# nexus-xyz/nexus-zkvm

Measured on AMD Instinct MI355X. Metric: RISC-V cycles proved/sec at log_n_rows=22; achieved HBM GB/s on Circle-FFT, higher is better.
Workload: dtype u32 (M31); 1 GPU; synthetic 2^22-row trace, full prove (LDE+quotient+FRI+Merkle), 27 preprocessed + 347 main + 64 interaction columns (16 real logup columns generated on device, recorded AIR), blowup 2, 3 queries, pow_bits 10, standard Blake2s-256 Merkle nodes; log_n_rows=22, parallelism=1 GPU, proof_words=11971

## Files before the change

### nexus-zkvm_amd/csrc/ctx.hip

```cpp
#include "internal.h"
#include <execinfo.h>
#include <signal.h>
#include <unistd.h>
#include <string.h>
#include <stdlib.h>
#include <algorithm>
#include <thread>

namespace nx {

thread_local std::string g_last_error;

int set_err(nx_ctx* ctx, int code, const std::string& msg) {
    g_last_error = msg;
    if (ctx) ctx->err = msg;
    return code;
}
int hip_fail(nx_ctx* ctx, hipError_t e, const char* what, const char* file, int line) {
    char buf[512];
    snprintf(buf, sizeof buf, "HIP error %d (%s) in `%s` at %s:%d", (int)e, hipGetErrorString(e), what, file, line);
    return set_err(ctx, e == hipErrorOutOfMemory ? NX_ERR_OOM : NX_ERR_HIP, buf);
}

int stage(nx_ctx* ctx, const void* h_src, size_t bytes, void** d_out) {
// ... 214 lines not shown

__global__ __launch_bounds__(256) void transpose_blocks_kernel(uint32_t* full, uint64_t col_stride, uint32_t* blocks, uint32_t n_cols, uint64_t rows, uint32_t world, int unpack) {
    const uint64_t rb4 = rows / world / 4, total = (uint64_t)n_cols * world * rb4;
    for (uint64_t i = blockIdx.x * (uint64_t)blockDim.x + threadIdx.x; i < total; i += (uint64_t)gridDim.x * blockDim.x) {
        const uint64_t x = i % rb4, cd = i / rb4;
        const uint32_t c = (uint32_t)(cd % n_cols), d = (uint32_t)(cd / n_cols);
        uint4* f = reinterpret_cast<uint4*>(full + (uint64_t)c * col_stride) + (uint64_t)d * rb4 + x;
        uint4* b = reinterpret_cast<uint4*>(blocks) + ((uint64_t)d * n_cols + c) * rb4 + x;
        if (unpack) *f = *b; else *b = *f;
    }
}
int transpose_blocks(nx_ctx* ctx, uint32_t* full, uint64_t col_stride, uint32_t* blocks, uint32_t n_cols, uint64_t rows, uint32_t world, bool unpack) {
    if (!n_cols || !rows) return NX_OK;
    if ((rows / world) % 4 || rows % world || col_stride % 4) return set_err(ctx, NX_ERR_ARG, "transpose_blocks: the row block must be a multiple of 4 words");
    const uint64_t total = (uint64_t)n_cols * rows / 4;
    hipLaunchKernelGGL(transpose_blocks_kernel, dim3((unsigned)std::min<uint64_t>((total + 255) / 256, (uint64_t)ctx->n_cus * 32)), dim3(256), 0, ctx->stream, full, col_stride, blocks, n_cols,
                       rows, world, unpack ? 1 : 0);
    NX_LAUNCH_CHECK(ctx);
    return NX_OK;
}

}

using namespace nx;

__global__ __launch_bounds__(256) void copy_cols_kernel(nx::ColSet dst, nx::ColSet src, size_t n4) {
    const uint4* __restrict__ s = (const uint4*)src.col(blockIdx.y);
    uint4* __restrict__ d = (uint4*)dst.col(blockIdx.y);
    for (size_t i = (size_t)blockIdx.x * 256 + threadIdx.x; i < n4; i += (size_t)gridDim.x * 256) d[i] = s[i];
}
namespace nx {
int copy_columns(nx_ctx* ctx, uint32_t* const* h_dst, const uint32_t* const* h_src, uint32_t n_cols, size_t n_words) {
    if (n_cols == 0 || n_words == 0) return NX_OK;
    bool vec = (n_words & 3) == 0;
    for (uint32_t k = 0; k < n_cols && vec; k++) vec = !(((uintptr_t)h_dst[k] | (uintptr_t)h_src[k]) & 15);
    if (!vec || n_cols < 4) { for (uint32_t k = 0; k < n_cols; k++) NX_TRY(nx_copy(ctx, h_dst[k], h_src[k], n_words)); return NX_OK; }
    for (uint32_t c0 = 0; c0 < n_cols; c0 += 65535) {
        const uint32_t nb = std::min<uint32_t>(65535, n_cols - c0);
        ColSet d, s;
        NX_TRY(make_colset(ctx, h_dst + c0, nb, &d));
        NX_TRY(make_colset(ctx, (uint32_t* const*)(h_src + c0), nb, &s));
        const size_t n4 = n_words / 4;
        const unsigned bx = (unsigned)std::max<size_t>(1, std::min<size_t>((n4 + 255) / 256, std::max<size_t>(1, (size_t)ctx->n_cus * 16 / nb)));
        hipLaunchKernelGGL(copy_cols_kernel, dim3(bx, nb), dim3(256), 0, ctx->stream, d, s, n4);
        NX_LAUNCH_CHECK(ctx);
    }
    return NX_OK;
}
}

extern "C" {

const char* nx_version(void) { return "nexus_hip 0.3 (gfx950)"; }

const char* nx_last_error(const nx_ctx* ctx) { return ctx ? ctx->err.c_str() : g_last_error.c_str(); }

static int env_int(const char* name, int dflt) { const char* e = getenv(name); return e ? atoi(e) : dflt; }
static int clampi(int v, int lo, int hi) { return v < lo ? lo : v > hi ? hi : v; }
static nx_options options_from_env() {
    nx_options o;
    o.fft_batch_cols = std::max(1, env_int("NX_FFT_BATCH", 2));
    o.fft_streams = clampi(env_int("NX_FFT_STREAMS", 2), 1, 4);
    o.fri_dist_min_log = std::max(0, env_int("NX_FRI_DIST_MIN_LOG", 21));
    o.dist_chunks = std::max(0, env_int("NX_DIST_CHUNKS", 0));
    o.air_segment = std::max(200, env_int("NX_AIR_SEGMENT", 9000));
    o.air_degree_split = env_int("NX_AIR_DEGREE_SPLIT", 1) != 0;
    o.quotients_coeffs = env_int("NX_QUOTIENTS_COEFFS", 1) != 0;
    o.air_half_domain = env_int("NX_AIR_HALF_DOMAIN", 1) != 0;
    o.air_quarter_domain = std::max(0, std::min(2, env_int("NX_AIR_QUARTER_DOMAIN", 2)));
    o.comm_timeout_ms = std::max(0, env_int("NX_COMM_TIMEOUT_MS", 120000));
    o.fft_kmax = clampi(env_int("NX_FFT_KMAX", 9), 1, 11);
    o.fft_fused = env_int("NX_FFT_FUSED", 1) != 0;
    o.merkle_fused = clampi(env_int("NX_MERKLE_FUSED", 21), 0, 31);
    o.merkle_subtree = clampi(env_int("NX_MERKLE_SUBTREE", 14), 0, 30);
    o.merkle_top = clampi(env_int("NX_MERKLE_TOP", 7), 1, 10);
    o.merkle_pair_levels = env_int("NX_MERKLE_PAIR_LEVELS", 1) != 0;
    o.fri_device_channel = env_int("NX_FRI_DEVICE_CHANNEL", 1) != 0;
    o.fri_tail = clampi(env_int("NX_FRI_TAIL", 1), 0, 11);
    o.logup_scan_tiled = env_int("NX_LOGUP_SCAN_TILED", 1) != 0;
    o.logup_per_column = env_int("NX_LOGUP_PER_COLUMN", 0) != 0;
    o.machine_reuse_pre = env_int("NX_MACHINE_REUSE_PREPROCESSED", 0) != 0;
    o.machine_logup_program = env_int("NX_MACHINE_LOGUP_PROGRAM", 0) != 0;
    o.trace_vec4 = env_int("NX_TRACE_VEC4", 1) != 0;
    o.host_pack_threads = clampi((int)std::thread::hardware_concurrency(), 1, 16);
    return o;
}
struct OptEntry { const char* name; int nx_options::*field; int lo, hi; };
static const OptEntry k_options[] = {
    {"fft.batch_cols", &nx_options::fft_batch_cols, 1, 256},
    {"fft.streams", &nx_options::fft_streams, 1, 4},
    {"fri.dist_min_log", &nx_options::fri_dist_min_log, 0, 31},
    {"dist.chunks", &nx_options::dist_chunks, 0, 64},
    {"air.segment", &nx_options::air_segment, 200, 1 << 30},
    {"air.degree_split", &nx_options::air_degree_split, 0, 1},
    {"quotients.coeffs", &nx_options::quotients_coeffs, 0, 1},
    {"air.half_domain", &nx_options::air_half_domain, 0, 1},
    {"air.quarter_domain", &nx_options::air_quarter_domain, 0, 2},
    {"comm.timeout_ms", &nx_options::comm_timeout_ms, 0, 1 << 30},
    {"fft.kmax", &nx_options::fft_kmax, 1, 11},
    {"fft.fused", &nx_options::fft_fused, 0, 1},
    {"merkle.fused", &nx_options::merkle_fused, 0, 31},
    {"merkle.subtree", &nx_options::merkle_subtree, 0, 30},
    {"merkle.top", &nx_options::merkle_top, 1, 10},
    {"merkle.pair_levels", &nx_options::merkle_pair_levels, 0, 1},
    {"fri.device_channel", &nx_options::fri_device_channel, 0, 1},
    {"fri.tail", &nx_options::fri_tail, 0, 11},
    {"logup.scan_tiled", &nx_options::logup_scan_tiled, 0, 1},
    {"logup.per_column", &nx_options::logup_per_column, 0, 1},
    {"machine.reuse_preprocessed", &nx_options::machine_reuse_pre, 0, 1},
    {"machine.logup_program", &nx_options::machine_logup_program, 0, 1},
    {"trace.vec4", &nx_options::trace_vec4, 0, 1},
    {"host.pack_threads", &nx_options::host_pack_threads, 1, 64},
};
int nx_ctx_set_option(nx_ctx* ctx, const char* name, int64_t value) {
    if (!ctx || !name) return set_err(ctx, NX_ERR_ARG, "nx_ctx_set_option: NULL argument");
    for (const OptEntry& e : k_options)
        if (!strcmp(e.name, name)) {
            if (value < e.lo || value > e.hi) return set_err(ctx, NX_ERR_ARG, std::string("nx_ctx_set_option: value out of range for ") + name);
            ctx->opt.*(e.field) = (int)value;
            return NX_OK;
        }
    return set_err(ctx, NX_ERR_ARG, std::string("nx_ctx_set_option: unknown option ") + name);
}
int nx_ctx_get_option(const nx_ctx* ctx, const char* name, int64_t* value) {
    if (!ctx || !name || !value) return set_err(const_cast<nx_ctx*>(ctx), NX_ERR_ARG, "nx_ctx_get_option: NULL argument");
    for (const OptEntry& e : k_options)
        if (!strcmp(e.name, name)) { *value = ctx->opt.*(e.field); return NX_OK; }
    return set_err(const_cast<nx_ctx*>(ctx), NX_ERR_ARG, std::string("nx_ctx_get_option: unknown option ") + name);
}

static void abort_backtrace(int sig) {
    void* frames[64];
    const int n = backtrace(frames, 64);
    static const char msg[] = "\n[nexus_hip] SIGABRT — native stack of the aborting thread:\n";
    (void)!write(2, msg, sizeof msg - 1);
    backtrace_symbols_fd(frames, n, 2);
    signal(sig, SIG_DFL);
    raise(sig);
}
int nx_ctx_create(int device, nx_ctx** out) {
    if (!out) return set_err(nullptr, NX_ERR_ARG, "nx_ctx_create: out is NULL");
    { static bool once = false; if (!once) { once = true; const char* e = getenv("NX_ABORT_BACKTRACE"); if (e && *e == '1') signal(SIGABRT, abort_backtrace); } }
    int count = 0;
    hipError_t e = hipGetDeviceCount(&count);
    if (e != hipSuccess || count <= 0)
        return set_err(nullptr, NX_ERR_NO_DEVICE, "nx_ctx_create: no HIP device visible (this library has no CPU fallback)");
    if (device < 0 || device >= count) return set_err(nullptr, NX_ERR_ARG, "nx_ctx_create: bad device index");
    hipDeviceProp_t prop;
    NX_HIP(nullptr, hipGetDeviceProperties(&prop, device));
    if (!strstr(prop.gcnArchName, "gfx950"))
        return set_err(nullptr, NX_ERR_NO_DEVICE, std::string("nx_ctx_create: device is ") + prop.gcnArchName + ", this library is built for gfx950 only");
    NX_HIP(nullptr, hipSetDevice(device));
    nx_ctx* c = new nx_ctx();
    c->opt = options_from_env();
    c->device = device; c->hash_mode = NX_HASH_BLAKE2S; c->timing = false; c->n_cus = prop.multiProcessorCount > 0 ? prop.multiProcessorCount : 256;
    c->scratch_size = 16u << 20; c->scratch_off = 0; c->d_scratch = nullptr; c->h_scratch = nullptr; c->cached_bytes = 0;
    for (int i = 0; i < 4; i++) { c->kind_ms[i] = 0; c->kind_bytes[i] = 0; }
    NX_HIP(nullptr, hipStreamCreateWithFlags(&c->stream, hipStreamNonBlocking));
    c->cur = c->stream;
    NX_HIP(nullptr, hipStreamCreateWithFlags(&c->copy_stream, hipStreamNonBlocking));
    NX_HIP(nullptr, hipStreamCreateWithFlags(&c->perm_stream, hipStreamNonBlocking));
    NX_HIP(nullptr, hipEventCreateWithFlags(&c->fork_ev, hipEventDisableTiming));
    for (int i = 0; i < 3; i++) {
        NX_HIP(nullptr, hipStreamCreateWithFlags(&c->side[i], hipStreamNonBlocking));
        NX_HIP(nullptr, hipEventCreateWithFlags(&c->join_ev[i], hipEventDisableTiming));
    }
    NX_HIP(nullptr, hipMalloc((void**)&c->d_scratch, c->scratch_size));
    NX_HIP(nullptr, hipHostMalloc((void**)&c->h_scratch, c->scratch_size, hipHostMallocDefault));
    *out = c;
    return NX_OK;
}

void nx_ctx_destroy(nx_ctx* ctx) {
    NX_GUARD(ctx);
    if (!ctx) return;
    (void)hipSetDevice(ctx->device);
    (void)hipStreamSynchronize(ctx->stream);
    nxhip::machine_kernels_release(ctx);
    nx::logup_kernels_release(ctx);
    timing_flush(ctx);
    for (auto e : ctx->event_pool) (void)hipEventDestroy(e);
    dev_cache_release(ctx);
    for (auto& kv : ctx->live_blocks) (void)hipFree(kv.first);
    if (ctx->d_scratch) (void)hipFree(ctx->d_scratch);
    if (ctx->h_scratch) (void)hipHostFree(ctx->h_scratch);
    if (ctx->h_bounce) { (void)hipHostFree(ctx->h_bounce); for (int k = 0; k < 2; k++) (void)hipEventDestroy(ctx->bounce_ev[k]); }
    pack_ring_release(ctx);
    for (auto& kv : ctx->free_pinned) (void)hipHostFree(kv.second);
    for (auto& kv : ctx->live_pinned) (void)hipHostFree(kv.first);
    for (int i = 0; i < 3; i++) { (void)hipStreamDestroy(ctx->side[i]); (void)hipEventDestroy(ctx->join_ev[i]); }
    (void)hipEventDestroy(ctx->fork_ev);
    (void)hipStreamDestroy(ctx->copy_stream); (void)hipStreamDestroy(ctx->perm_stream);
    (void)hipStreamDestroy(ctx->stream);
    delete ctx;
}

int nx_ctx_set_hash_mode(nx_ctx* ctx, int mode) {
    if (!ctx) return set_err(nullptr, NX_ERR_ARG, "nx_ctx_set_hash_mode: NULL context");
    if (mode != NX_HASH_BLAKE2S && mode != NX_HASH_BLAKE2S_RAW0) return set_err(ctx, NX_ERR_ARG, "bad hash mode");
    ctx->hash_mode = mode;
    return NX_OK;
}

int nx_sync(nx_ctx* ctx) { NX_GUARD(ctx); if (!ctx) return set_err(nullptr, NX_ERR_ARG, "nx_sync: NULL context"); NX_HIP(ctx, hipStreamSynchronize(ctx->stream)); return NX_OK; }
int nx_ctx_trim(nx_ctx* ctx) { NX_GUARD(ctx); if (!ctx) return set_err(nullptr, NX_ERR_ARG, "nx_ctx_trim: NULL context"); NX_TRY(nx_sync(ctx)); dev_cache_release(ctx); pack_ring_release(ctx); return NX_OK; }
void* nx_ctx_stream(nx_ctx* ctx) { return ctx ? (void*)ctx->stream : nullptr; }
int nx_ctx_memory(nx_ctx* ctx, uint64_t* live_bytes, uint64_t* peak_bytes, int reset_peak) {
    if (!ctx) return set_err(nullptr, NX_ERR_ARG, "nx_ctx_memory: NULL context");
    if (live_bytes) *live_bytes = ctx->live_bytes;
    if (peak_bytes) *peak_bytes = ctx->peak_live_bytes;
    if (reset_peak) ctx->peak_live_bytes = ctx->live_bytes;
    return NX_OK;
}

int nx_alloc(nx_ctx* ctx, size_t n_words, uint32_t** d_out) {
    NX_GUARD(ctx);
    if (!ctx || !d_out) return set_err(ctx, NX_ERR_ARG, "nx_alloc: NULL argument");
    *d_out = nullptr;
    return dev_alloc(ctx, n_words * 4, (void**)d_out);
}
int nx_free(nx_ctx* ctx, uint32_t* d_ptr) {
    NX_GUARD(ctx);
    if (!ctx) return set_err(nullptr, NX_ERR_ARG, "nx_free: NULL context");
    dev_free(ctx, d_ptr);
    return NX_OK;
}
int nx_memset_zero(nx_ctx* ctx, uint32_t* d_ptr, size_t n_words) {
    NX_GUARD(ctx);
    if (!ctx || (!d_ptr && n_words)) return set_err(ctx, NX_ERR_ARG, "nx_memset_zero: NULL argument");
    if (!n_words) return NX_OK;
    NX_HIP(ctx, hipMemsetAsync(d_ptr, 0, n_words * 4, ctx->stream));
    return NX_OK;
}
int nx_upload(nx_ctx* ctx, uint32_t* d_dst, const uint32_t* h_src, size_t n_words) {
    NX_GUARD(ctx);
    if (!ctx || ((!d_dst || !h_src) && n_words)) return set_err(ctx, NX_ERR_ARG, "nx_upload: NULL argument");
    if (!n_words) return NX_OK;
    return copy_h2d_blocking(ctx, d_dst, h_src, n_words * 4);
}
int nx_download(nx_ctx* ctx, uint32_t* h_dst, const uint32_t* d_src, size_t n_words) {
    NX_GUARD(ctx);
    if (!ctx || ((!h_dst || !d_src) && n_words)) return set_err(ctx, NX_ERR_ARG, "nx_download: NULL argument");
    if (!n_words) return NX_OK;
    return copy_d2h_blocking(ctx, h_dst, d_src, n_words * 4);
}

int nx_copy(nx_ctx* ctx, uint32_t* d_dst, const uint32_t* d_src, size_t n_words) {
    NX_GUARD(ctx);
    if (!ctx || ((!d_dst || !d_src) && n_words)) return set_err(ctx, NX_ERR_ARG, "nx_copy: NULL argument");
    if (n_words == 0) return NX_OK;
    if ((n_words & 3) || ((uintptr_t)d_dst & 15) || ((uintptr_t)d_src & 15)) {
        NX_HIP(ctx, hipMemcpyAsync(d_dst, d_src, n_words * 4, hipMemcpyDeviceToDevice, ctx->stream));
        return NX_OK;
    }
    size_t n4 = n_words / 4;
    unsigned blocks = (unsigned)std::min<size_t>((n4 + 255) / 256, (size_t)ctx->n_cus * 16);
    hipLaunchKernelGGL(copy_kernel, dim3(blocks), dim3(256), 0, ctx->stream, (uint4*)d_dst, (const uint4*)d_src, n4);
    NX_LAUNCH_CHECK(ctx);
    return NX_OK;
}

static unsigned stream_grid(nx_ctx* ctx, size_t n) { return (unsigned)std::min<size_t>((n + 255) / 256, (size_t)ctx->n_cus * 16); }
int nx_m31_add_into(nx_ctx* ctx, uint32_t* d_dst, const uint32_t* d_src, size_t n_words) {
    NX_GUARD(ctx);
    if (!n_words) return NX_OK;
    hipLaunchKernelGGL(m31_add_into_kernel, dim3(stream_grid(ctx, n_words)), dim3(256), 0, ctx->stream, d_dst, d_src, n_words);
    NX_LAUNCH_CHECK(ctx);
    return NX_OK;
}
int nx_m31_widen(nx_ctx* ctx, uint64_t* d_dst, const uint32_t* d_src, size_t n_words) {
    NX_GUARD(ctx);
    if (!n_words) return NX_OK;
    hipLaunchKernelGGL(m31_widen_kernel, dim3(stream_grid(ctx, n_words)), dim3(256), 0, ctx->stream, (u64*)d_dst, d_src, n_words);
    NX_LAUNCH_CHECK(ctx);
    return NX_OK;
}
int nx_m31_narrow(nx_ctx* ctx, uint32_t* d_dst, const uint64_t* d_src, size_t n_words) {
    NX_GUARD(ctx);
    if (!n_words) return NX_OK;
    hipLaunchKernelGGL(m31_narrow_kernel, dim3(stream_grid(ctx, n_words)), dim3(256), 0, ctx->stream, d_dst, (const u64*)d_src, n_words);
    NX_LAUNCH_CHECK(ctx);
    return NX_OK;
}

int nx_gather(nx_ctx* ctx, const uint32_t* const* d_ptrs, const uint64_t* index, size_t n, uint32_t* h_out) {
    NX_GUARD(ctx);
    if (!ctx || ((!d_ptrs || !index || !h_out) && n)) return set_err(ctx, NX_ERR_ARG, "nx_gather: NULL argument");
    if (n == 0) return NX_OK;
// ... 24 lines not shown
```

### nexus-zkvm_amd/csrc/fft.hip

```cpp
#include "internal.h"
#include "host/narrow_pack.h"
#include <mutex>
#include <atomic>
#include <stdlib.h>
#include <algorithm>

namespace nx {

__global__ void twiddle_kernel(u32* tw, u32* itw, int h, GenTable gen) {
    u32 p = blockIdx.x * blockDim.x + threadIdx.x;
    u32 total = 1u << h;
    if (p >= total) return;
    u32 q = total - p;
    u32 val;
    if (q == 1) {
        val = 1;
    } else {
        int m = 31 - __clz(q - 1);
        int l = h - 1 - m;
        u32 k = (2u << m) - q;
        u32 init = (1u << (31 - h - 2)) << l, step = (1u << (31 - h)) << l;
        u32 idx = (init + step * bitrev(k, m)) & 0x7fffffffu;
        val = pt_from_index_tbl(gen, idx).x;
    }
// ... 250 lines not shown
}

static int check_tw(nx_ctx* ctx, const nx_twiddles* tw, int n) {
    if (!tw) return set_err(ctx, NX_ERR_ARG, "twiddles are NULL");
    if (n < 1 || n - 1 > (int)tw->log_half) return set_err(ctx, NX_ERR_ARG, "domain larger than the twiddle tree (or log_size < 1)");
    return NX_OK;
}

static int interpolate_cols(nx_ctx* ctx, const nx_twiddles* tw, ColSet cols, u32 n_cols, int n) {
    if (n >= 13 && !g_tune.legacy) return fft13_interpolate(ctx, tw, cols, n_cols, n);
    if (n <= 2) {
        hipLaunchKernelGGL(fft_tiny_kernel, dim3((n_cols + 63) / 64), dim3(64), 0, ctx->cur, cols, cols, n_cols, n, n, true);
        NX_LAUNCH_CHECK(ctx);
        return NX_OK;
    }
    std::vector<PassPlan> plan = plan_passes(n);
    u32 scale = m_inv(1u << n);
    for (size_t i = 0; i < plan.size(); i++) {
        FftPass a; a.src = cols; a.dst = cols; a.tw = tw->d_itw; a.tw_log = tw->log_half; a.n = n; a.log_in = n;
        a.lo = plan[i].lo; a.hi = plan[i].hi; a.B = plan[i].B; a.scale = i + 1 == plan.size() ? scale : 0; a.n_cols = n_cols;
        NX_TRY(launch_pass(ctx, true, a));
    }
    return NX_OK;
}

static int evaluate_cols(nx_ctx* ctx, const nx_twiddles* tw, ColSet polys, u32 n_cols, int log_in, int n, ColSet out) {
    if (log_in >= 13 && !g_tune.legacy) return fft13_evaluate(ctx, tw, polys, n_cols, log_in, n, out);
    if (n <= 2) {
        hipLaunchKernelGGL(fft_tiny_kernel, dim3((n_cols + 63) / 64), dim3(64), 0, ctx->cur, polys, out, n_cols, n, log_in, false);
        NX_LAUNCH_CHECK(ctx);
        return NX_OK;
    }
    std::vector<PassPlan> plan = plan_passes(n);
    for (size_t k = plan.size(); k-- > 0;) {
        bool first = k + 1 == plan.size();
        FftPass a; a.src = first ? polys : out; a.dst = out; a.tw = tw->d_tw; a.tw_log = tw->log_half; a.n = n;
        a.log_in = first ? log_in : n; a.lo = plan[k].lo; a.hi = plan[k].hi; a.B = plan[k].B; a.scale = 0; a.n_cols = n_cols;
        NX_TRY(launch_pass(ctx, false, a));
    }
    return NX_OK;
}

static u32 batch_for(const nx_ctx* ctx, uint32_t log_size) {
    if (log_size > 22) return (u32)std::max(1, ctx->opt.fft_batch_cols >> std::min<uint32_t>(log_size - 22, 8));
    const int shift = log_size < 22 ? (int)(22 - log_size) : 0;
    return (u32)std::min<uint64_t>((uint64_t)ctx->opt.fft_batch_cols << std::min(shift, 8), 256);
}

int fft_interpolate(nx_ctx* ctx, const nx_twiddles* tw, ColSet cols, uint32_t n_cols, uint32_t log_size) {
    NX_TRY(check_tw(ctx, tw, (int)log_size));
    tune_init();
    KTimer t(ctx, NX_T_LDE, (uint64_t)n_cols * 8ull << log_size);
    const u32 bc = batch_for(ctx, log_size);
    const int ns = n_cols > bc ? ctx->opt.fft_streams : 1;
    NX_TRY(streams_fork(ctx, ns));
    int rc = NX_OK;
    for (u32 c0 = 0, bi = 0; c0 < n_cols && rc == NX_OK; c0 += bc, bi++) {
        u32 nb = std::min<u32>(bc, n_cols - c0);
        streams_pick(ctx, (int)bi, ns);
        rc = interpolate_cols(ctx, tw, sub_colset(cols, c0), nb, (int)log_size);
    }
    int rj = streams_join(ctx, ns);
    return rc != NX_OK ? rc : rj;
}

int fft_evaluate(nx_ctx* ctx, const nx_twiddles* tw, ColSet polys, uint32_t n_cols, uint32_t log_size, uint32_t log_expand, ColSet out) {
    int n = (int)(log_size + log_expand);
    NX_TRY(check_tw(ctx, tw, n));
    tune_init();
    KTimer t(ctx, NX_T_LDE, (uint64_t)n_cols * ((4ull << log_size) + (4ull << n)));
    const u32 bc = batch_for(ctx, log_size);
    const int ns = n_cols > bc ? ctx->opt.fft_streams : 1;
    NX_TRY(streams_fork(ctx, ns));
    int rc = NX_OK;
    for (u32 c0 = 0, bi = 0; c0 < n_cols && rc == NX_OK; c0 += bc, bi++) {
        u32 nb = std::min<u32>(bc, n_cols - c0);
        streams_pick(ctx, (int)bi, ns);
        rc = evaluate_cols(ctx, tw, sub_colset(polys, c0), nb, (int)log_size, n, sub_colset(out, c0));
    }
    int rj = streams_join(ctx, ns);
    return rc != NX_OK ? rc : rj;
}

int fft_lde(nx_ctx* ctx, const nx_twiddles* tw, ColSet cols, uint32_t n_cols, uint32_t log_size, uint32_t log_expand, ColSet out) {
    int n = (int)(log_size + log_expand);
    NX_TRY(check_tw(ctx, tw, n));
    tune_init();
    KTimer t(ctx, NX_T_LDE, (uint64_t)n_cols * ((8ull << log_size) + (4ull << n)));
    const u32 bc = batch_for(ctx, log_size);
    const int ns = n_cols > bc ? ctx->opt.fft_streams : 1;
    NX_TRY(streams_fork(ctx, ns));
    int rc = NX_OK;
    for (u32 c0 = 0, bi = 0; c0 < n_cols && rc == NX_OK; c0 += bc, bi++) {
        u32 nb = std::min<u32>(bc, n_cols - c0);
        streams_pick(ctx, (int)bi, ns);
        if (log_expand == 1 && log_size >= 14 && ctx->opt.fft_fused) {
            rc = fft13_lde(ctx, tw, sub_colset(cols, c0), nb, (int)log_size, sub_colset(out, c0));
            continue;
        }
        rc = interpolate_cols(ctx, tw, sub_colset(cols, c0), nb, (int)log_size);
        if (rc == NX_OK) rc = evaluate_cols(ctx, tw, sub_colset(cols, c0), nb, (int)log_size, n, sub_colset(out, c0));
    }
    int rj = streams_join(ctx, ns);
    return rc != NX_OK ? rc : rj;
}

__global__ void bit_reverse_kernel(u32* col, int log) {
    u32 i = blockIdx.x * blockDim.x + threadIdx.x;
    if (i >= (1u << log)) return;
    u32 j = bitrev(i, log);
    if (i < j) { u32 a = col[i], b = col[j]; col[i] = b; col[j] = a; }
}

__device__ __forceinline__ u32 natural_index_of(u32 i, int log) {
    u32 N = 1u << log, d = bitrev(i, log);
    return d < N / 2 ? 2 * d : 2 * N - 1 - 2 * d;
}
__global__ void finalize_kernel(ColSet src, ColSet dst, u32 n_cols, int log) {
    u32 i = blockIdx.x * blockDim.x + threadIdx.x;
    u32 c = blockIdx.y;
    if (i >= (1u << log) || c >= n_cols) return;
    dst.col(c)[i] = src.col(c)[natural_index_of(i, log)];
}

template <int W, bool PERMUTE>
__global__ void __launch_bounds__(256) widen_kernel(const uint8_t* __restrict__ src, uint32_t* __restrict__ dst, int log, int vec) {
    const u32 i = blockIdx.x * blockDim.x + threadIdx.x, n = 1u << log;
    auto at = [&](u32 j) -> u32 { return W == 1 ? (u32)src[j] : (u32)((const uint16_t*)src)[j]; };
    if (PERMUTE) { if (i < n) dst[i] = at(natural_index_of(i, log)); return; }
    constexpr u32 E = 16 / W;
    if (!vec) { if (i < n) dst[i] = at(i); return; }
    if (i >= n / E) return;
    const uint4 v = gld4((const uint32_t*)(src + (size_t)i * 16));
    uint32_t* d = dst + (size_t)i * E;
    const u32 w[4] = {v.x, v.y, v.z, v.w};
#pragma unroll
    for (int q = 0; q < 4; q++) {
        if (W == 1) gst4(d + 4 * q, make_uint4(w[q] & 0xffu, (w[q] >> 8) & 0xffu, (w[q] >> 16) & 0xffu, w[q] >> 24));
        else if (q < 2) gst4(d + 4 * q, make_uint4(w[2 * q] & 0xffffu, w[2 * q] >> 16, w[2 * q + 1] & 0xffffu, w[2 * q + 1] >> 16));
    }
}

__global__ void twiddle_double_kernel(const u32* tw, const u32* itw, u32* tw2, u32* itw2, u32 n) {
    u32 i = blockIdx.x * blockDim.x + threadIdx.x;
    if (i < n) { tw2[i] = tw[i] << 1; itw2[i] = itw[i] << 1; }
}

}

using namespace nx;

extern "C" {

int nx_twiddles_create(nx_ctx* ctx, uint32_t log_half_coset, nx_twiddles** out) {
    NX_GUARD(ctx);
    if (!ctx || !out) return set_err(ctx, NX_ERR_ARG, "nx_twiddles_create: NULL argument");
    if (log_half_coset < 1 || log_half_coset > 28) return set_err(ctx, NX_ERR_ARG, "nx_twiddles_create: log_half_coset out of range [1,28]");
    nx_twiddles* t = new nx_twiddles();
    t->ctx = ctx; t->log_half = log_half_coset; t->d_tw = nullptr; t->d_itw = nullptr; t->d_tw2 = nullptr; t->d_itw2 = nullptr;
    size_t bytes = (size_t)4 << log_half_coset;
    int rc0 = dev_alloc(ctx, bytes, (void**)&t->d_tw);
    if (rc0 == NX_OK) rc0 = dev_alloc(ctx, bytes, (void**)&t->d_itw);
    if (rc0 == NX_OK) rc0 = dev_alloc(ctx, bytes, (void**)&t->d_tw2);
    if (rc0 == NX_OK) rc0 = dev_alloc(ctx, bytes, (void**)&t->d_itw2);
    if (rc0 != NX_OK) { dev_free(ctx, t->d_tw); dev_free(ctx, t->d_itw); dev_free(ctx, t->d_tw2); dev_free(ctx, t->d_itw2); delete t; return rc0; }
    hipError_t e;
    u32 total = 1u << log_half_coset;
    const GenTable gen = gen_table();
    hipLaunchKernelGGL(twiddle_kernel, dim3((total + 255) / 256), dim3(256), 0, ctx->stream, t->d_tw, t->d_itw, (int)log_half_coset, gen);
    hipLaunchKernelGGL(twiddle_double_kernel, dim3((total + 255) / 256), dim3(256), 0, ctx->stream, t->d_tw, t->d_itw, t->d_tw2, t->d_itw2, total);
    e = hipGetLastError();
    if (e != hipSuccess) { dev_free(ctx, t->d_tw); dev_free(ctx, t->d_itw); dev_free(ctx, t->d_tw2); dev_free(ctx, t->d_itw2); delete t; return hip_fail(ctx, e, "twiddle_kernel", __FILE__, __LINE__); }
    *out = t;
    return NX_OK;
}

}
namespace nx {
__global__ void sub_twiddle_kernel(const u32* __restrict__ s0, const u32* __restrict__ s1, const u32* __restrict__ s2, const u32* __restrict__ s3,
                                   u32* __restrict__ d0, u32* __restrict__ d1, u32* __restrict__ d2, u32* __restrict__ d3, int n, int L, int depth) {
    const u32 i = blockIdx.x * blockDim.x + threadIdx.x, half = 1u << (n - 1);
    if (i >= half) return;
    if (i + 1 == half) { d0[i] = 1; d1[i] = 1; d2[i] = 2; d3[i] = 2; return; }
    const u32 m = half - i;
    const int K = 32 - __builtin_clz(m - 1);
    const u32 h = (1u << K) - m;
    const u32 src = (1u << L) - (1u << (K + depth)) + h;
    d0[i] = s0[src]; d1[i] = s1[src]; d2[i] = s2[src]; d3[i] = s3[src];
}
int twiddles_first_part(nx_ctx* ctx, const nx_twiddles* tw, uint32_t n, uint32_t depth, nx_twiddles** out) {
    if (depth < 1 || depth > 4 || n < 3 || n + depth - 1 > tw->log_half) return set_err(ctx, NX_ERR_ARG, "twiddles_first_part: need 1 <= depth <= 4 and 3 <= n <= log_half + 1 - depth of the source tree");
    nx_twiddles* t = new nx_twiddles();
    t->ctx = ctx; t->log_half = n - 1; t->d_tw = t->d_itw = t->d_tw2 = t->d_itw2 = nullptr;
    const size_t bytes = (size_t)4 << (n - 1);
    int rc = dev_alloc(ctx, bytes, (void**)&t->d_tw);
    if (rc == NX_OK) rc = dev_alloc(ctx, bytes, (void**)&t->d_itw);
    if (rc == NX_OK) rc = dev_alloc(ctx, bytes, (void**)&t->d_tw2);
    if (rc == NX_OK) rc = dev_alloc(ctx, bytes, (void**)&t->d_itw2);
    if (rc != NX_OK) { dev_free(ctx, t->d_tw); dev_free(ctx, t->d_itw); dev_free(ctx, t->d_tw2); dev_free(ctx, t->d_itw2); delete t; return rc; }
    const u32 half = 1u << (n - 1);
    hipLaunchKernelGGL(sub_twiddle_kernel, dim3((half + 255) / 256), dim3(256), 0, ctx->stream, tw->d_tw, tw->d_itw, tw->d_tw2, tw->d_itw2, t->d_tw, t->d_itw, t->d_tw2, t->d_itw2,
                       (int)n, (int)tw->log_half, (int)depth);
    if (hipGetLastError() != hipSuccess) { nx_twiddles_destroy(t); return set_err(ctx, NX_ERR_HIP, "sub_twiddle_kernel launch failed"); }
    *out = t;
    return NX_OK;
}
}
extern "C" {

void nx_twiddles_destroy(nx_twiddles* tw) {
    NX_GUARD(tw ? tw->ctx : nullptr);
    if (!tw) return;
    dev_free(tw->ctx, tw->d_tw); dev_free(tw->ctx, tw->d_itw); dev_free(tw->ctx, tw->d_tw2); dev_free(tw->ctx, tw->d_itw2);
    delete tw;
}

int nx_twiddles_download(nx_ctx* ctx, const nx_twiddles* tw, uint32_t* h_tw, uint32_t* h_itw) {
    NX_GUARD(ctx);
    if (!ctx || !tw || !h_tw || !h_itw) return set_err(ctx, NX_ERR_ARG, "nx_twiddles_download: NULL argument");
    NX_TRY(nx_download(ctx, h_tw, tw->d_tw, (size_t)1 << tw->log_half));
    return nx_download(ctx, h_itw, tw->d_itw, (size_t)1 << tw->log_half);
}

int nx_interpolate_batch(nx_ctx* ctx, const nx_twiddles* tw, uint32_t* const* d_cols, uint32_t n_cols, uint32_t log_size) {
    NX_GUARD(ctx);
    if (n_cols == 0) return NX_OK;
    ColSet cs; NX_TRY(make_colset(ctx, d_cols, n_cols, &cs));
    return fft_interpolate(ctx, tw, cs, n_cols, log_size);
}

int nx_evaluate_batch(nx_ctx* ctx, const nx_twiddles* tw, const uint32_t* const* d_polys, uint32_t n_cols, uint32_t log_size,
                      uint32_t log_expand, uint32_t* const* d_out) {
    NX_GUARD(ctx);
    if (n_cols == 0) return NX_OK;
    ColSet p, o;
    NX_TRY(make_colset(ctx, d_polys, n_cols, &p));
    NX_TRY(make_colset(ctx, d_out, n_cols, &o));
    return fft_evaluate(ctx, tw, p, n_cols, log_size, log_expand, o);
}

int nx_bit_reverse(nx_ctx* ctx, uint32_t* d_col, uint32_t log_size) {
    NX_GUARD(ctx);
    if (!ctx || !d_col) return set_err(ctx, NX_ERR_ARG, "nx_bit_reverse: NULL argument");
    if (log_size > 31) return set_err(ctx, NX_ERR_ARG, "nx_bit_reverse: log_size too large");
    u32 n = 1u << log_size;
    hipLaunchKernelGGL(bit_reverse_kernel, dim3((n + 255) / 256), dim3(256), 0, ctx->stream, d_col, (int)log_size);
    NX_LAUNCH_CHECK(ctx);
    return NX_OK;
}

int nx_finalize_columns(nx_ctx* ctx, const uint32_t* const* d_src_natural, uint32_t* const* d_dst, uint32_t n_cols, uint32_t log_size) {
    NX_GUARD(ctx);
    if (n_cols == 0) return NX_OK;
    if (log_size < 1) return set_err(ctx, NX_ERR_ARG, "nx_finalize_columns: log_size < 1");
    ColSet s, d;
    NX_TRY(make_colset(ctx, d_src_natural, n_cols, &s));
    NX_TRY(make_colset(ctx, d_dst, n_cols, &d));
    u32 n = 1u << log_size;
    for (u32 c0 = 0; c0 < n_cols; c0 += 32768) {
        u32 nb = std::min<u32>(32768, n_cols - c0);
        hipLaunchKernelGGL(finalize_kernel, dim3((n + 255) / 256, nb), dim3(256), 0, ctx->stream, sub_colset(s, c0), sub_colset(d, c0), nb, (int)log_size);
        NX_LAUNCH_CHECK(ctx);
    }
    return NX_OK;
}

}
namespace nx {
int HostFeed::begin(nx_ctx* c, uint32_t log_size, int coset) {
    ctx = c; log = log_size; coset_order = coset; n_done = n_slot = n_packed = 0;
    if (log_size < 1 || log_size > 30) return set_err(c, NX_ERR_ARG, "host feed: bad log_size");
    for (int k = 0; k < 2; k++) {
        if (coset_order) NX_TRY(dev_alloc(ctx, (size_t)4 << log, (void**)&d_tmp[k]));
        NX_HIP(ctx, hipEventCreateWithFlags(&copied[k], hipEventDisableTiming));
        NX_HIP(ctx, hipEventCreateWithFlags(&consumed[k], hipEventDisableTiming));
    }
    hipEvent_t here = nullptr;
    NX_HIP(ctx, hipEventCreateWithFlags(&here, hipEventDisableTiming));
    events.push_back(here);
    NX_HIP(ctx, hipEventRecord(here, ctx->stream));
    NX_HIP(ctx, hipStreamWaitEvent(ctx->copy_stream, here, 0));
    NX_HIP(ctx, hipStreamWaitEvent(ctx->perm_stream, here, 0));
    return NX_OK;
}
static int kind_width(uint8_t kind) { return kind == NX_COL_U8 || kind == NX_COL_U32_AS_U8 ? 1 : kind == NX_COL_U16 || kind == NX_COL_U32_AS_U16 ? 2 : 4; }
static const char* kind_name(uint8_t kind) {
    static const char* const names[] = {"NX_COL_U32", "NX_COL_U16", "NX_COL_U8", "NX_COL_U32_AS_U16", "NX_COL_U32_AS_U8"};
    return kind <= NX_COL_U32_AS_U8 ? names[kind] : "an unknown kind";
}
static int pack_ring_reserve(nx_ctx* ctx, size_t bytes) {
    if (ctx->pack_bytes >= bytes) return NX_OK;
    pack_ring_release(ctx);
    for (int s = 0; s < 2; s++) {
        NX_HIP(ctx, hipEventCreateWithFlags(&ctx->pack_ev[s], hipEventDisableTiming));
        NX_HIP(ctx, hipEventRecord(ctx->pack_ev[s], ctx->copy_stream));
// ... 233 lines not shown
```

### nexus-zkvm_amd/csrc/fft13.hip

```cpp
#include "internal.h"
#include <atomic>
#include <algorithm>
#include <stdlib.h>

namespace nx {

#ifndef NX_FFT_MINWAVES
#define NX_FFT_MINWAVES 1
#endif
#ifndef NX_FFT_MINWAVES1
#define NX_FFT_MINWAVES1 1
#endif
constexpr int T13_S = 13;
constexpr u32 T13_ROWS = 1u << T13_S;
constexpr u32 T13_HALF = T13_ROWS / 2;

struct Pass13 {
    ColSet src, dst;
    const u32* tw;
    u32 tw_log;
    int n;
    int log_in;
    int lo, K, B;
    u32 scale;
// ... 485 lines not shown
    const size_t lds_bytes = ((size_t)T13_ROWS + (T13_ROWS >> 4)) * 4 * CB;
    if (!(attr_set.load() & (1ull << (ctx->device & 63)))) {
        NX_HIP(ctx, hipFuncSetAttribute((const void*)fft13_kernel<INV, FIRST, CB, RB, KT>, hipFuncAttributeMaxDynamicSharedMemorySize, 160 * 1024));
        attr_set.fetch_or(1ull << (ctx->device & 63));
    }
    dim3 grid(a.tiles * a.n_groups), block(T13_ROWS >> RB);
    hipLaunchKernelGGL((fft13_kernel<INV, FIRST, CB, RB, KT>), grid, block, lds_bytes, ctx->cur, a);
    NX_LAUNCH_CHECK(ctx);
    return NX_OK;
}

template <bool INV, int CB, int RB>
static int launch13_k(nx_ctx* ctx, bool first, const Pass13& a) {
    if (first) return launch13_t<INV, true, CB, RB, 0>(ctx, a);
    switch (a.K) {
    case 1: return launch13_t<INV, false, CB, RB, 1>(ctx, a);
    case 2: return launch13_t<INV, false, CB, RB, 2>(ctx, a);
    case 3: return launch13_t<INV, false, CB, RB, 3>(ctx, a);
    case 4: return launch13_t<INV, false, CB, RB, 4>(ctx, a);
    case 5: return launch13_t<INV, false, CB, RB, 5>(ctx, a);
    case 6: return launch13_t<INV, false, CB, RB, 6>(ctx, a);
    case 7: return launch13_t<INV, false, CB, RB, 7>(ctx, a);
    case 8: return launch13_t<INV, false, CB, RB, 8>(ctx, a);
    case 9: return launch13_t<INV, false, CB, RB, 9>(ctx, a);
    default: return launch13_t<INV, false, CB, RB, 0>(ctx, a);
    }
}

static int launch13(nx_ctx* ctx, bool inv, bool first, Pass13 a) {
    a.n_groups = a.n_cols;
    return inv ? launch13_k<true, 1, 4>(ctx, first, a) : launch13_k<false, 1, 4>(ctx, first, a);
}

int fft13_interpolate(nx_ctx* ctx, const nx_twiddles* tw, ColSet cols, u32 n_cols, int n) {
    std::vector<Plan13> plan = plan13(n, ctx->opt.fft_kmax);
    for (size_t i = 0; i < plan.size(); i++) {
        Pass13 a; a.src = cols; a.dst = cols; a.tw = tw->d_itw2; a.tw_log = tw->log_half; a.n = n; a.log_in = n;
        a.lo = plan[i].lo; a.K = plan[i].K; a.B = plan[i].B; a.scale = i + 1 == plan.size() ? m_inv(1u << n) : 0;
        a.n_cols = n_cols; a.n_groups = 0; a.tiles = 1u << (n - T13_S); a.rep_log = 0;
        NX_TRY(launch13(ctx, true, i == 0, a));
    }
    return NX_OK;
}

int fft13_evaluate(nx_ctx* ctx, const nx_twiddles* tw, ColSet polys, u32 n_cols, int log_in, int n, ColSet out) {
    std::vector<Plan13> plan = plan13(log_in, ctx->opt.fft_kmax);
    for (size_t k = plan.size(); k-- > 0;) {
        const bool top = k + 1 == plan.size();
        Pass13 a; a.src = top ? polys : out; a.dst = out; a.tw = tw->d_tw2; a.tw_log = tw->log_half; a.n = n; a.log_in = top ? log_in : n;
        a.lo = plan[k].lo; a.K = plan[k].K; a.B = plan[k].B; a.scale = 0;
        a.n_cols = n_cols; a.n_groups = 0; a.tiles = 1u << (n - T13_S); a.rep_log = top ? (u32)(n - log_in) : 0;
        NX_TRY(launch13(ctx, false, k == 0, a));
    }
    return NX_OK;
}

template <int RB, int KT>
static int launch_mid_t(nx_ctx* ctx, const PassMid& m) {
    static std::atomic<uint64_t> attr_set{0};
    const size_t lds_bytes = ((size_t)T13_ROWS + (T13_ROWS >> 4)) * 4 * 2;
    if (!(attr_set.load() & (1ull << (ctx->device & 63)))) {
        NX_HIP(ctx, hipFuncSetAttribute((const void*)lde_mid_kernel<RB, KT>, hipFuncAttributeMaxDynamicSharedMemorySize, 160 * 1024));
        attr_set.fetch_or(1ull << (ctx->device & 63));
    }
    hipLaunchKernelGGL((lde_mid_kernel<RB, KT>), dim3(m.tiles * m.n_cols), dim3(T13_ROWS >> RB), lds_bytes, ctx->cur, m);
    NX_LAUNCH_CHECK(ctx);
    return NX_OK;
}
static int launch_mid(nx_ctx* ctx, const PassMid& m) {
    switch (m.K) {
    case 1: return launch_mid_t<4, 1>(ctx, m);
    case 2: return launch_mid_t<4, 2>(ctx, m);
    case 3: return launch_mid_t<4, 3>(ctx, m);
    case 4: return launch_mid_t<4, 4>(ctx, m);
    case 5: return launch_mid_t<4, 5>(ctx, m);
    case 6: return launch_mid_t<4, 6>(ctx, m);
    case 7: return launch_mid_t<4, 7>(ctx, m);
    case 8: return launch_mid_t<4, 8>(ctx, m);
    case 9: return launch_mid_t<4, 9>(ctx, m);
    default: return launch_mid_t<4, 0>(ctx, m);
    }
}

int fft13_lde(nx_ctx* ctx, const nx_twiddles* tw, ColSet cols, u32 n_cols, int n, ColSet out) {
    std::vector<Plan13> plan = plan13(n, ctx->opt.fft_kmax);
    const size_t P = plan.size();
    if (P < 2) return set_err(ctx, NX_ERR_ARG, "fft13_lde: needs at least two passes");
    for (size_t i = 0; i + 1 < P; i++) {
        Pass13 a; a.src = cols; a.dst = cols; a.tw = tw->d_itw2; a.tw_log = tw->log_half; a.n = n; a.log_in = n;
        a.lo = plan[i].lo; a.K = plan[i].K; a.B = plan[i].B; a.scale = 0;
        a.n_cols = n_cols; a.n_groups = 0; a.tiles = 1u << (n - T13_S); a.rep_log = 0;
        NX_TRY(launch13(ctx, true, i == 0, a));
    }
    {
        PassMid m; m.cols = cols; m.out = out; m.itw = tw->d_itw2; m.tw = tw->d_tw2; m.tw_log = tw->log_half; m.n = n;
        m.lo = plan[P - 1].lo; m.K = plan[P - 1].K; m.B = plan[P - 1].B; m.scale = m_inv(1u << n); m.n_cols = n_cols; m.tiles = 1u << (n - T13_S);
        NX_TRY(launch_mid(ctx, m));
    }
    for (size_t k = P - 1; k-- > 0;) {
        Pass13 a; a.src = out; a.dst = out; a.tw = tw->d_tw2; a.tw_log = tw->log_half; a.n = n + 1; a.log_in = n + 1;
        a.lo = plan[k].lo; a.K = plan[k].K; a.B = plan[k].B; a.scale = 0;
        a.n_cols = n_cols; a.n_groups = 0; a.tiles = 1u << (n + 1 - T13_S); a.rep_log = 0;
        NX_TRY(launch13(ctx, false, k == 0, a));
    }
    return NX_OK;
}

}
```

### nexus-zkvm_amd/csrc/internal.h

```cpp
#pragma once
#include <hip/hip_runtime.h>
#include <stdint.h>
#include <stdio.h>
#include <string>
#include <vector>
#include <map>
#include <memory>
#include "../../include/nexus_hip.h"
#include "field.cuh"

struct nx_options {
    int fft_batch_cols;
    int fft_streams;
    int fri_dist_min_log;
    int dist_chunks;
    int air_segment;
    int quotients_coeffs;
    int air_half_domain;
    int air_quarter_domain;
    int comm_timeout_ms;
    int fft_kmax;
    int fft_fused;
    int merkle_fused;
    int merkle_top;
    int merkle_subtree; int merkle_pair_levels;
    int fri_device_channel;
    int fri_tail;
    int logup_scan_tiled;
    int logup_per_column;
    int machine_logup_program;
    int machine_reuse_pre;
    int air_degree_split;
    int trace_vec4;
    int host_pack_threads;
};

struct nx_ctx {
    int device;
    nx_options opt;
    hipStream_t stream;
    hipStream_t side[3];
    hipEvent_t fork_ev, join_ev[3];
    hipStream_t cur;
    hipStream_t copy_stream, perm_stream;
    int hash_mode;
    int n_cus;
    std::string err;
    uint8_t* d_scratch;
    size_t scratch_size, scratch_off;
    uint8_t* h_scratch;
    uint8_t* h_bounce = nullptr; hipEvent_t bounce_ev[2] = {nullptr, nullptr};
    uint8_t* h_pack[2] = {nullptr, nullptr}; size_t pack_bytes = 0; hipEvent_t pack_ev[2] = {nullptr, nullptr};
    std::multimap<size_t, void*> free_blocks;
    std::map<void*, size_t> live_blocks;
    size_t cached_bytes;
    size_t live_bytes = 0, peak_live_bytes = 0;
    std::multimap<size_t, void*> free_pinned;
    std::map<void*, size_t> live_pinned;
    bool timing;
    struct Span { hipEvent_t e0, e1; int kind; };
    std::vector<Span> spans;
    std::vector<hipEvent_t> event_pool;
    double kind_ms[4];
    uint64_t kind_bytes[4];
    std::vector<uint32_t> last_claimed;
    bool symmetric_failure = false;
    bool comm_entered = false;
    std::map<std::string, std::shared_ptr<void>> machine_pre_cache;
};
enum { NX_T_LDE = 0, NX_T_MERKLE = 1, NX_T_QUOT = 2, NX_T_OTHER = 3 };

struct nx_twiddles {
    nx_ctx* ctx;
    uint32_t log_half;
    uint32_t* d_tw;
    uint32_t* d_itw;
    uint32_t* d_tw2;
    uint32_t* d_itw2;
};

struct nx_tree {
    nx_ctx* ctx;
    std::vector<uint32_t*> layers;
};

namespace nx { void logup_kernels_release(nx_ctx* ctx); }
namespace nxhip { void machine_kernels_release(nx_ctx* ctx); }
namespace nxhip {
double now_ms();
bool host_prof_on();
void host_prof_add(const char* name, double ms);
void host_prof_dump(const char* title);
struct HostSpan {
    const char* name; double t0; bool live;
    explicit HostSpan(const char* n) : name(n), t0(host_prof_on() ? now_ms() : 0), live(host_prof_on()) {}
    void stop() { if (live) { host_prof_add(name, now_ms() - t0); live = false; } }
    ~HostSpan() { stop(); }
    HostSpan(const HostSpan&) = delete;
    HostSpan& operator=(const HostSpan&) = delete;
};
}

namespace nx {

extern thread_local std::string g_last_error;

int set_err(nx_ctx* ctx, int code, const std::string& msg);
int hip_fail(nx_ctx* ctx, hipError_t e, const char* what, const char* file, int line);

#define NX_HIP(ctx, call)                                                         \
    do {                                                                          \
        hipError_t e__ = (call);                                                  \
        if (e__ != hipSuccess) return nx::hip_fail((ctx), e__, #call, __FILE__, __LINE__); \
    } while (0)
#define NX_TRY(call)                  \
    do {                              \
        int rc__ = (call);            \
        if (rc__ != NX_OK) return rc__; \
    } while (0)
#define NX_LAUNCH_CHECK(ctx) NX_HIP(ctx, hipGetLastError())

struct DeviceGuard {
    int prev = -1; bool switched = false;
    explicit DeviceGuard(const nx_ctx* c) {
        if (!c) return;
        if (hipGetDevice(&prev) != hipSuccess) { prev = -1; }
        if (prev != c->device) { switched = hipSetDevice(c->device) == hipSuccess && prev >= 0; }
    }
    ~DeviceGuard() { if (switched) (void)hipSetDevice(prev); }
    DeviceGuard(const DeviceGuard&) = delete;
    DeviceGuard& operator=(const DeviceGuard&) = delete;
};
#define NX_GUARD(ctxexpr) nx::DeviceGuard nx_device_guard__(ctxexpr)

struct ColSet {
    uint32_t* base;
    uint64_t stride;
    uint32_t* const* table;
    __device__ __forceinline__ uint32_t* col(uint32_t c) const { return table ? table[c] : base + (uint64_t)c * stride; }
};

#if defined(__HIP_DEVICE_COMPILE__) || defined(__HIPCC__)
#define NX_GLOBAL_AS __attribute__((address_space(1)))
typedef uint32_t nx_v4u32 __attribute__((ext_vector_type(4)));
__device__ __forceinline__ uint32_t gld(const uint32_t* p) { return *(NX_GLOBAL_AS const uint32_t*)p; }
__device__ __forceinline__ uint32_t gld_off(const uint32_t* base, uint32_t byte_off) { return *(NX_GLOBAL_AS const uint32_t*)((NX_GLOBAL_AS const char*)base + byte_off); }
__device__ __forceinline__ uint4 gld4(const uint32_t* p) { const nx_v4u32 v = *(NX_GLOBAL_AS const nx_v4u32*)p; return make_uint4(v.x, v.y, v.z, v.w); }
__device__ __forceinline__ void gst(uint32_t* p, uint32_t v) { *(NX_GLOBAL_AS uint32_t*)p = v; }
__device__ __forceinline__ void gst4(uint32_t* p, uint4 v) { nx_v4u32 w = {v.x, v.y, v.z, v.w}; *(NX_GLOBAL_AS nx_v4u32*)p = w; }
#endif

template <class T> static inline T* bias_rows(T* p, uint64_t row_begin) { return p ? (T*)((uintptr_t)p - row_begin * sizeof(T)) : p; }

int make_colset(nx_ctx* ctx, const uint32_t* const* h_ptrs, uint32_t n, ColSet* out);
int stage(nx_ctx* ctx, const void* h_src, size_t bytes, void** d_out);
int host_alloc(nx_ctx* ctx, size_t bytes, void** h_out);
void host_free(nx_ctx* ctx, void* p);
struct EvalJob { uint8_t* blob; const uint32_t* h_part; uint32_t np, n_chunks; std::vector<uint32_t> evals; uint32_t* h_out; };
int eval_at_points_enqueue(nx_ctx* ctx, const uint32_t* const* d_polys, uint32_t log_size, const uint32_t* poly_idx, const uint32_t* h_points, uint32_t n_evals,
                           uint32_t* h_out, std::vector<EvalJob>* jobs);
int eval_at_points_collect(nx_ctx* ctx, std::vector<EvalJob>* jobs);
int dev_alloc(nx_ctx* ctx, size_t bytes, void** out);
void dev_free(nx_ctx* ctx, void* p);
void dev_cache_release(nx_ctx* ctx);

int copy_columns(nx_ctx* ctx, uint32_t* const* h_dst, const uint32_t* const* h_src, uint32_t n_cols, size_t n_words);
bool host_pinned_by_owner(const void* p, size_t bytes);
int copy_h2d_blocking(nx_ctx* ctx, void* d_dst, const void* h_src, size_t bytes, hipStream_t stream = nullptr);
int copy_d2h_blocking(nx_ctx* ctx, void* h_dst, const void* d_src, size_t bytes);
int upload_async_staged(nx_ctx* ctx, void* d_dst, const void* h_src, size_t bytes);
void pack_ring_release(nx_ctx* ctx);
int upload_columns(nx_ctx* ctx, const void* const* h_cols, const uint8_t* kinds, uint32_t n_cols, uint32_t log_size, uint32_t* const* d_cols,
                   int coset_order, const uint32_t* call_col, const char* what);
struct HostFeed {
    nx_ctx* ctx = nullptr; int coset_order = 0; uint32_t log = 0;
    uint32_t* d_tmp[2] = {nullptr, nullptr}; hipEvent_t copied[2] = {nullptr, nullptr}, consumed[2] = {nullptr, nullptr};
    uint64_t n_done = 0, n_slot = 0, n_packed = 0;
    std::vector<const void*> pinned; std::vector<hipEvent_t> events;
    int begin(nx_ctx* c, uint32_t log_size, int coset);
    int chunk(const void* const* h_cols, const uint8_t* kinds, const uint32_t* call_col, const char* what, uint32_t* const* d_cols, uint32_t n_cols, hipEvent_t* ready);
    int finish();
    ~HostFeed() { (void)finish(); }
};
int transpose_blocks(nx_ctx* ctx, uint32_t* full, uint64_t col_stride, uint32_t* blocks, uint32_t n_cols, uint64_t rows, uint32_t world, bool unpack);

struct KTimer {
    nx_ctx* ctx; int idx;
    KTimer(nx_ctx* c, int kind, uint64_t algorithmic_bytes);
    ~KTimer();
};
void timing_flush(nx_ctx* ctx);
void timing_reset(nx_ctx* ctx);

int fft_interpolate(nx_ctx* ctx, const nx_twiddles* tw, ColSet cols, uint32_t n_cols, uint32_t log_size);
int fft_evaluate(nx_ctx* ctx, const nx_twiddles* tw, ColSet polys, uint32_t n_cols, uint32_t log_size,
                 uint32_t log_expand, ColSet out);

constexpr int FRI_TAIL_LOG = 11, FRI_TAIL_MAX_LAYERS = 16;
int tree_alloc(nx_ctx* ctx, uint32_t max_log, nx_tree** out);
constexpr int FRI_STATE_HEAD = 9, FRI_STATE_REC = 12;
int merkle_commit_fused(nx_ctx* ctx, const uint32_t* const* d_cols, uint32_t n_cols, uint32_t log, nx_tree** out);
int fri_fold_commit_fused(nx_ctx* ctx, const nx_twiddles* tw, const uint32_t* const* d_src4, uint32_t src_log, const uint32_t* d_alpha, uint32_t* const* d_dst4, nx_tree** out);
int fri_channel_step(nx_ctx* ctx, uint32_t* d_state, const uint32_t* d_root, int j);
int fri_tail(nx_ctx* ctx, const nx_twiddles* tw, uint32_t* const* evals, uint32_t* const* trees, int n_layers, int log0, uint32_t* d_state, int j0);
int fold_circle_dev(nx_ctx* ctx, const nx_twiddles* tw, uint32_t* const* d_dst4, const uint32_t* const* d_src4, uint32_t src_log, const uint32_t* d_alpha);
int fold_line_dev(nx_ctx* ctx, const nx_twiddles* tw, const uint32_t* const* d_src4, uint32_t src_log, const uint32_t* d_alpha, uint32_t* const* d_dst4);
int fold_circle_rows(nx_ctx* ctx, const nx_twiddles* tw, uint32_t* const* d_dst4, const uint32_t* const* d_src4, uint32_t src_log, const uint32_t alpha[4], uint32_t i0, uint32_t n);
int fold_line_rows(nx_ctx* ctx, const nx_twiddles* tw, const uint32_t* const* d_src4, uint32_t src_log, const uint32_t alpha[4], uint32_t* const* d_dst4, uint32_t i0, uint32_t n);
int accumulate_quotients_rows(nx_ctx* ctx, uint32_t log_size, const uint32_t* const* d_cols, uint32_t n_cols, const uint32_t random_coeff[4], uint32_t n_batches,
                              const uint32_t* points, const uint32_t* batch_counts, const uint32_t* col_idx, const uint32_t* values, uint32_t* const* d_out4,
                              uint64_t row_begin, uint64_t n_rows);
int twiddles_first_part(nx_ctx* ctx, const nx_twiddles* tw, uint32_t n, uint32_t depth, nx_twiddles** out);
inline int twiddles_first_half(nx_ctx* ctx, const nx_twiddles* tw, uint32_t n, nx_twiddles** out) { return twiddles_first_part(ctx, tw, n, 1, out); }
int accumulate_quotients_coeffs(nx_ctx* ctx, const nx_twiddles* tw, uint32_t log_size, uint32_t log_coef, const uint32_t* const* d_polys, uint32_t n_cols,
                                const uint32_t random_coeff[4], uint32_t n_batches, const uint32_t* points, const uint32_t* batch_counts, const uint32_t* col_idx,
                                const uint32_t* values, uint32_t* const* d_out4);

struct TreePipe {
    nx_tree* tree = nullptr;
    uint32_t max_log = 0, total_leaf_cols = 0, absorbed = 0;
    std::vector<const uint32_t*> pending;
    bool any_launch = false;
};
int tree_pipe_begin(nx_ctx* ctx, uint32_t max_log, uint32_t total_leaf_cols, TreePipe* tp);
int tree_pipe_absorb(nx_ctx* ctx, TreePipe* tp, const uint32_t* const* d_cols, uint32_t n_cols, bool flush);
int tree_pipe_finish(nx_ctx* ctx, TreePipe* tp, const uint32_t* const* d_small_cols, const uint32_t* small_logs, uint32_t n_small, nx_tree** out);
int leaf_chain_launch(nx_ctx* ctx, ColSet cs, uint32_t n_cols, uint32_t col_offset, uint32_t total_cols, const uint32_t* state_in, uint32_t* state_out, uint64_t row_begin, uint64_t n_rows);
int fft_lde(nx_ctx* ctx, const nx_twiddles* tw, ColSet cols, uint32_t n_cols, uint32_t log_size, uint32_t log_expand, ColSet out);

int streams_fork(nx_ctx* ctx, int n_streams);
void streams_pick(nx_ctx* ctx, int batch_index, int n_streams);
int streams_join(nx_ctx* ctx, int n_streams);

int fft13_interpolate(nx_ctx* ctx, const nx_twiddles* tw, ColSet cols, uint32_t n_cols, int n);
int fft13_evaluate(nx_ctx* ctx, const nx_twiddles* tw, ColSet polys, uint32_t n_cols, int log_in, int n, ColSet out);
int fft13_lde(nx_ctx* ctx, const nx_twiddles* tw, ColSet cols, uint32_t n_cols, int n, ColSet out);


}
```

### nexus-zkvm_amd/csrc/machine.hip

```cpp
#include "prover.h"
#include <mutex>
#include <array>

namespace nxhip {

struct Loc { size_t pre0, main0, inter0; };

static std::vector<Loc> locations(const nx_component_spec* comps, uint32_t n_comps, uint32_t* max_log) {
    std::vector<Loc> locs; size_t a = 0, b = 0, c = 0; *max_log = 0;
    for (uint32_t i = 0; i < n_comps; i++) { locs.push_back({a, b, c}); a += comps[i].n_pre; b += comps[i].n_main; c += comps[i].n_inter; *max_log = std::max(*max_log, comps[i].log_size); }
    return locs;
}

static QM31 synth_eval_composition_at_point(const nx_component_spec* comps, uint32_t n_comps, const std::vector<Loc>& locs, QPt point,
                                            const SampledValues& sv, QM31 random_coeff) {
    QM31 acc = q_zero();
    for (uint32_t ci = 0; ci < n_comps; ci++) {
        const nx_component_spec& c = comps[ci];
        QM31 di = q_inv(coset_vanishing_q(c.log_size, point));
        auto add = [&](QM31 v) { acc = q_add(q_mul(acc, random_coeff), q_mul(di, v)); };
        auto M = [&](uint32_t k, int s = 0) { return sv[1][locs[ci].main0 + k][s]; };
        auto I = [&](uint32_t k) { return sv[2][locs[ci].inter0 + k][0]; };
        QM31 not_last = q_sub(q_one(), sv[0][locs[ci].pre0 + 1][0]);
        add(q_mul(q_sub(q_sub(M(0, 1), M(0)), q_one()), not_last));
// ... 40 lines not shown
        for (uint32_t ci = 0; ci < n_comps; ci++) {
            const nx_component_spec& c = comps[ci];
            const uint32_t e = c.log_size + comp_log_cd(c.log_constraint_degree_bound, cs.cfg);
            std::vector<std::pair<uint32_t, uint32_t>> cc;
            for (uint32_t k = 0; k < c.n_pre; k++) cc.push_back({0u, (uint32_t)locs[ci].pre0 + k});
            for (uint32_t k = 0; k < c.n_main; k++) cc.push_back({1u, (uint32_t)locs[ci].main0 + k});
            for (uint32_t k = 0; k < c.n_inter; k++) cc.push_back({2u, (uint32_t)locs[ci].inter0 + k});
            std::vector<char> masked(cc.size(), 0);
            masked[c.n_pre] = masked[c.n_pre + 1] = 1;
            EvalDomainCols cols;
            H_TRY(columns_on_eval_domain(cs, cc, c.log_size, e, masked, &cols));
            ColSet pre, mainc, inter;
            H_TRY(make_colset(ctx, cols.ptrs.data(), c.n_pre, &pre));
            H_TRY(make_colset(ctx, cols.ptrs.data() + c.n_pre, c.n_main, &mainc));
            H_TRY(make_colset(ctx, cols.ptrs.data() + c.n_pre + c.n_main, c.n_inter, &inter));
            SecureColumn* acc = nullptr;
            H_TRY(composition_accumulator(cs, sub, e, &acc));
            const uint64_t rb = cs.dist.on() ? cs.dist.begin(e) : 0;
            u32* a4[4]; for (int k = 0; k < 4; k++) a4[k] = bias_rows(acc->c[k], rb);
            SynthRange rg{0, c.n_main, c.n_main, 0, c.n_inter, true};
            H_TRY(synth_constraints(ctx, pre, mainc, inter, rg, (int)c.log_size, (int)e, d_params.p + off_pw[ci], d_params.p + off_den[ci], a4, (u32)rb, (u32)acc->rows));
        }
        return finalize_accumulation(cs, sub, out_polys, out_log);
    }
    void mask_points(QPt oods, MaskPoints* points) override {
        points->assign(3, {});
        for (uint32_t i = 0; i < n_comps; i++) {
            QPt step; { Pt s = pt_from_index(1u << (31 - comps[i].log_size)); step.x = q_from_m(s.x); step.y = q_from_m(s.y); }
            for (uint32_t k = 0; k < comps[i].n_pre; k++) (*points)[0].push_back({oods});
            for (uint32_t k = 0; k < comps[i].n_main; k++) { if (k < 2) (*points)[1].push_back({oods, qpt_add(oods, step)}); else (*points)[1].push_back({oods}); }
            for (uint32_t k = 0; k < comps[i].n_inter; k++) (*points)[2].push_back({oods});
        }
    }
    QM31 eval_composition_at_point(QPt point, const SampledValues& sv, QM31 rc) override { return synth_eval_composition_at_point(comps, n_comps, locs, point, sv, rc); }
};

static int check_components(nx_ctx* ctx, const nx_component_spec* comps, uint32_t n_comps, const nx_pcs_config* ucfg) {
    if (n_comps == 0) return set_err(ctx, NX_ERR_ARG, "prove: no components");
    if (ucfg->log_blowup < 1 || ucfg->log_constraint_degree < 1 || ucfg->log_constraint_degree > 2) return set_err(ctx, NX_ERR_ARG, "prove: log_blowup >= 1 and log_constraint_degree in {1,2} required");
    for (uint32_t i = 0; i < n_comps; i++) {
        if (comps[i].n_pre < 2 || comps[i].n_main < 2 || comps[i].log_size < 1 || comps[i].log_size > 28) return set_err(ctx, NX_ERR_ARG, "synthetic component needs n_pre >= 2, n_main >= 2, 1 <= log_size <= 28");
        if (!comp_log_cd_ok(comps[i].log_constraint_degree_bound, ucfg->log_constraint_degree))
            return set_err(ctx, NX_ERR_ARG, "prove: a component's log_constraint_degree_bound exceeds the config's log_constraint_degree (the twiddle tree is sized by it)");
    }
    return NX_OK;
}

static int fill_and_extend(CommitmentSchemeProver& cs, TreeBuilder& tb, const nx_component_spec* comps, uint32_t n_comps, uint32_t tree, uint64_t seed, uint64_t inter_seed) {
    nx_ctx* ctx = cs.ctx;
    std::vector<std::pair<uint32_t, uint32_t>> groups, local;
    for (uint32_t i = 0; i < n_comps; i++) groups.push_back({tree == 0 ? comps[i].n_pre : tree == 1 ? comps[i].n_main : comps[i].n_inter, comps[i].log_size});
    plan_local_columns(groups, cs.dist, &local);
    for (uint32_t i = 0; i < n_comps; i++) {
        const uint32_t lo = local[i].first, hi = local[i].second, log = comps[i].log_size;
        DevBuf slab;
        if (hi > lo) {
            H_TRY(slab.alloc(ctx, (size_t)(hi - lo) << log));
            auto p = col_ptrs(slab.p, hi - lo, log);
            H_TRY(synth_fill_range(ctx, comps[i], i, tree, seed, inter_seed, lo, hi - lo, p.data(), 0, 1u << log));
        }
        tb.extend_evals_local(std::move(slab), groups[i].first, log, lo, hi);
    }
    return NX_OK;
}

static int prove_synth(nx_ctx* ctx, const nx_component_spec* comps, uint32_t n_comps, const nx_pcs_config* ucfg, uint64_t seed, const uint8_t* ad,
                       size_t ad_len, const nx_comm* comm, std::vector<uint32_t>* words, nx_prove_stats* st) {
    PcsConfig cfg = {ucfg->pow_bits, ucfg->log_blowup, ucfg->n_queries, ucfg->log_last_layer_degree_bound, ucfg->fri_alpha_mode, ucfg->log_constraint_degree};
    H_TRY(check_components(ctx, comps, n_comps, ucfg));
    for (uint32_t i = 0; i < n_comps; i++) if (comps[i].logup_mode) return set_err(ctx, NX_ERR_ARG, "nx_prove_synth: logup_mode is nx_prove_machine's (this machine's interaction trace is a synthetic fill)");
    H_TRY(nx_ctx_set_hash_mode(ctx, (int)ucfg->hash_mode));
    uint32_t max_log = 0;
    std::vector<Loc> locs = locations(comps, n_comps, &max_log);
    const bool timed = st != nullptr;
    nx_prove_stats local_stats;
    if (!st) st = &local_stats;
    memset(st, 0, sizeof *st);
    if (timed) { ctx->timing = true; timing_reset(ctx); }
    double t_start = 0;
    Lap lap{ctx, timed, 0};
    if (timed) { (void)nx_sync(ctx); t_start = lap.t0 = now_ms(); }

    nx_twiddles* tw = nullptr;
    H_TRY(nx_twiddles_create(ctx, max_log + cfg.log_constraint_degree + cfg.log_blowup - 1, &tw));
    struct TwGuard { nx_twiddles* t; ~TwGuard() { nx_twiddles_destroy(t); } } twg{tw};
    Blake2sChannel channel;
    for (size_t i = 0; i < ad_len; i++) channel.mix_u64(ad[i]);
    CommitmentSchemeProver cs(ctx, tw, cfg);
    if (comm) { H_TRY(dist_init(ctx, comm, &cs.dist)); cs.dist.comm_ms = &st->comm_ms; cs.dist.comm_bytes = &st->comm_bytes; cs.dist.comm_calls = &st->n_alltoallv; }
    for (uint32_t i = 0; i < n_comps; i++) channel.mix_u64(comps[i].log_size);
    lap(&st->commit);

    auto fill_and_commit = [&](uint32_t tree, uint64_t inter_seed) -> int {
        TreeBuilder tb = cs.tree_builder();
        H_TRY(fill_and_extend(cs, tb, comps, n_comps, tree, seed, inter_seed));
        lap(&st->trace_gen);
        H_TRY(tb.commit(channel));
        lap(&st->commit);
        return NX_OK;
    };
    H_TRY(fill_and_commit(0, 0));
    H_TRY(fill_and_commit(1, 0));
    QM31 z = channel.draw_secure_felt();
    uint64_t inter_seed = ((u64)z.a.a << 32) ^ (u64)z.a.b ^ ((u64)z.b.a << 16) ^ ((u64)z.b.b << 48);
    channel.mix_felts(std::vector<QM31>(n_comps, q_zero()));
    H_TRY(fill_and_commit(2, inter_seed));

    SynthAir air(comps, n_comps, locs);
    H_TRY(prove_core(ctx, cs, channel, cfg, tw, air, words, st, lap));
    if (timed) finish_stats(ctx, st, t_start);
    return NX_OK;
}

enum { E_COL = 0, E_CONST = 1, E_SUM = 2 };
enum { N_ONE = 0, N_NEG_MULT = 1, N_MULT_M1 = 2, N_ONE_M_MULT = 3, N_MULT = 4 };
struct TupleEntry { uint32_t kind, a, b; };
struct FracDef {
    bool table; uint32_t w, col[2]; bool has_mult; uint32_t mult;
    uint32_t num = N_ONE; std::vector<TupleEntry> ent;
};
static uint32_t tuple_sched(const nx_component_spec& c) { return (c.logup_mode >> 4) & 15u; }
static bool logup_mode_ok(uint32_t m) { return (m >> 4) <= NX_TUPLES_V2 && !((m & NX_LOGUP_ODD) && !(m & NX_LOGUP_PAIRS)) && !(m & 8u); }
static uint32_t n_logup_fracs(const nx_component_spec& c) {
    const uint32_t L = c.n_inter / 4;
    if (!(c.logup_mode & NX_LOGUP_PAIRS) || L == 0) return L;
    return 2 * L - ((c.logup_mode & NX_LOGUP_ODD) ? 1 : 0);
}
static FracDef frac_def(const nx_component_spec& c, uint32_t f) {
    FracDef d; d.table = (c.logup_mode & NX_LOGUP_TABLE) != 0;
    const uint32_t sched = tuple_sched(c), n = d.table ? c.n_pre : c.n_main;
    d.mult = (2 + 13 * f) % c.n_main;
    if (sched == 0) {
        d.w = (f & 1) ? 2 : 1;
        if (d.table) { d.col[0] = (2 + 3 * f) % c.n_pre; d.col[1] = (1 + 5 * f) % c.n_pre; d.has_mult = true; }
        else { d.col[0] = (3 + 7 * f) % c.n_main; d.col[1] = (5 + 11 * f) % c.n_main; d.has_mult = f % 3 == 2; }
        d.num = d.has_mult ? N_NEG_MULT : N_ONE;
        for (uint32_t k = 0; k < d.w; k++) d.ent.push_back({E_COL, d.col[k], 0});
        return d;
    }
    const uint32_t F = n_logup_fracs(c);
    static const uint32_t W1[8] = {1, 1, 4, 1, 9, 1, 3, 1}, W3[7] = {9, 21, 14, 10, 4, 12, 8};
    const bool state = sched == NX_TUPLES_KECCAK && !d.table && F >= 2 && f + 2 >= F;
    d.w = sched == NX_TUPLES_V1 ? W1[f % 8] : sched == NX_TUPLES_V2 ? W3[f % 7] : state ? 200 : (f % 4 == 3 ? 4 : 3);
    for (uint32_t k = 0; k < d.w; k++) d.ent.push_back({E_COL, ((d.table ? 2 + 3 * f : 3 + 7 * f) + 5 * k) % n, 0});
    auto sum = [&](uint32_t k) { d.ent[k].kind = E_SUM; d.ent[k].b = (5 + 11 * f + 3 * k) % n; };
    if (sched == NX_TUPLES_V1 && d.w == 4) d.ent[0] = {E_CONST, 1 + f % 3, 0};
    if (sched == NX_TUPLES_V1 && d.w == 3) { d.ent[1] = {E_CONST, 5, 0}; sum(2); }
    if (sched == NX_TUPLES_V2 && d.w == 4) { d.ent[1] = {E_CONST, 7, 0}; sum(2); }
    d.num = d.table ? N_NEG_MULT : f % 3 == 2 ? N_NEG_MULT : N_ONE;
    if (!d.table) {
        if (sched == NX_TUPLES_V1 && f % 8 == 2) d.num = N_MULT;
        if (sched == NX_TUPLES_V2 && f % 5 == 1 && f % 3 != 2) d.num = N_MULT;
        if (state) d.num = f + 2 == F ? N_MULT_M1 : N_ONE_M_MULT;
    }
    d.has_mult = d.num != N_ONE; d.col[0] = d.col[1] = 0;
    return d;
}
static uint32_t max_tuple_width(const nx_component_spec& c) {
    uint32_t w = 2;
    if (tuple_sched(c)) for (uint32_t f = 0; f < n_logup_fracs(c); f++) w = std::max(w, frac_def(c, f).w);
    return w;
}
static std::vector<uint32_t> batch_of(const nx_component_spec& c, uint32_t j) {
    if (!(c.logup_mode & NX_LOGUP_PAIRS)) return {j};
    std::vector<uint32_t> b{2 * j};
    if (2 * j + 1 < n_logup_fracs(c)) b.push_back(2 * j + 1);
    return b;
}
// ... 220 lines not shown
        const std::vector<nx_cinstr> prog = machine_fraction_program(c, &n_regs);
        hs_p.stop();
        const uint32_t n_cols = c.n_pre + c.n_main + c.n_inter;
        std::vector<const uint32_t*> cols(n_cols, nullptr);
        for (auto& kv : prev) cols[kv.first] = kv.second;
        for (auto& kv : mainv) cols[c.n_pre + kv.first] = kv.second;
        std::vector<uint32_t> ec(4 * (size_t)(APOW0 + max_tuple_width(c)), 0);
        fill_econsts(ec, z, alpha, q_zero());
        return nx_logup_program(ctx, prog.data(), (uint32_t)prog.size(), n_regs, cols.data(), n_cols, ec.data(), (uint32_t)(ec.size() / 4), log_rows, L, inter, nullptr);
    }
    std::vector<QM31> apow;
    { QM31 pw = q_one(); const QM31 al = q_load(alpha); for (uint32_t k = 0; k < max_tuple_width(c); k++) { apow.push_back(pw); pw = q_mul(pw, al); } }
    std::vector<std::vector<const uint32_t*>> tuples(F);
    std::vector<std::vector<uint32_t>> aps(F);
    std::vector<std::array<uint32_t, 4>> zs(F);
    std::vector<nx_logup_frac> fr(F);
    for (uint32_t f = 0; f < F; f++) {
        const FracDef& d = defs[f];
        const ColMap& src = d.table ? prev : mainv;
        QM31 zf = q_load(z);
        auto push = [&](uint32_t col, uint32_t k) { tuples[f].push_back(src.at(col)); aps[f].resize(aps[f].size() + 4); q_store(&aps[f][aps[f].size() - 4], apow[k]); };
        for (uint32_t k = 0; k < d.w; k++) {
            const TupleEntry& t = d.ent[k];
            if (t.kind == E_CONST) zf = q_sub(zf, q_mul_m(apow[k], t.a));
            else { push(t.a, k); if (t.kind == E_SUM) push(t.b, k); }
        }
        q_store(zs[f].data(), zf);
        nx_logup_frac& q = fr[f];
        q.d_tuple_cols = tuples[f].data(); q.n_tuple_cols = (uint32_t)tuples[f].size(); q.alpha_powers = aps[f].data(); q.z = zs[f].data();
        q.d_mult = d.has_mult ? mainv.at(d.mult) : nullptr; q.scale = d.num == N_NEG_MULT ? minus_one : one;
    }
    if (per_column) {
        for (uint32_t j = 0; j < L; j++) {
            const uint32_t f0 = pairs ? 2 * j : j;
            const nx_logup_frac* fb = pairs && f0 + 1 < F ? &fr[f0 + 1] : nullptr;
            H_TRY(nx_logup_col(ctx, log_rows, &fr[f0], fb, j ? (const uint32_t* const*)(inter + 4 * (j - 1)) : nullptr, inter + 4 * j));
        }
        return NX_OK;
    }
    if (pairs) return nx_logup_cols_batched(ctx, log_rows, fr.data(), F, nullptr, L, inter);
    return nx_logup_cols(ctx, log_rows, fr.data(), L, inter);
}
static std::set<uint32_t> logup_needed_columns(const nx_component_spec& c, uint32_t tree) {
    std::set<uint32_t> s;
    for (uint32_t f = 0; f < n_logup_fracs(c); f++) {
        const FracDef d = frac_def(c, f);
        if ((d.table ? 0u : 1u) == tree)
            for (const TupleEntry& t : d.ent) { if (t.kind != E_CONST) s.insert(t.a); if (t.kind == E_SUM) s.insert(t.b); }
        if (tree == 1 && d.has_mult) s.insert(d.mult);
    }
    return s;
}

struct HostTrace {
    const void* const* pre = nullptr; const void* const* main = nullptr; int coset_order = 0;
    const uint8_t* pre_kinds = nullptr; const uint8_t* main_kinds = nullptr;
};
static int prove_machine(nx_ctx* ctx, const nx_component_spec* comps, uint32_t n_comps, const nx_pcs_config* ucfg, uint64_t seed, const uint8_t* ad,
                         size_t ad_len, const nx_comm* comm, std::vector<uint32_t>* words, nx_prove_stats* st, const HostTrace* host = nullptr) {
    PcsConfig cfg = {ucfg->pow_bits, ucfg->log_blowup, ucfg->n_queries, ucfg->log_last_layer_degree_bound, ucfg->fri_alpha_mode, ucfg->log_constraint_degree};
    HostSpan hs_whole("pm.body (to the return statement)");
    HostSpan hs_pro("pm.prologue");
    H_TRY(check_components(ctx, comps, n_comps, ucfg));
    for (uint32_t i = 0; i < n_comps; i++) {
        if (comps[i].n_inter % 4) return set_err(ctx, NX_ERR_ARG, "nx_prove_machine: n_inter = 4 x (number of logup columns)");
        const uint32_t m = comps[i].logup_mode;
        if (!logup_mode_ok(m))
            return set_err(ctx, NX_ERR_ARG, "nx_prove_machine: logup_mode is a set of NX_LOGUP_PAIRS / NX_LOGUP_ODD (with PAIRS only) / NX_LOGUP_TABLE, plus NX_LOGUP_TUPLES(0 .. 3)");
    }
    H_TRY(nx_ctx_set_hash_mode(ctx, (int)ucfg->hash_mode));
    uint32_t max_log = 0;
    std::vector<Loc> locs = locations(comps, n_comps, &max_log);
    const bool timed = st != nullptr;
    nx_prove_stats local_stats;
    if (!st) st = &local_stats;
    memset(st, 0, sizeof *st);
    if (timed) { ctx->timing = true; timing_reset(ctx); }
    double t_start = 0;
    Lap lap{ctx, timed, 0};
    if (timed) { (void)nx_sync(ctx); t_start = lap.t0 = now_ms(); }

    hs_pro.stop();
    nx_twiddles* tw = nullptr;
    { HostSpan hs("pm.twiddles_create"); H_TRY(nx_twiddles_create(ctx, max_log + cfg.log_constraint_degree + cfg.log_blowup - 1, &tw)); }
    struct TwGuard { nx_twiddles* t; ~TwGuard() { nx_twiddles_destroy(t); } } twg{tw};
    Blake2sChannel channel;
    for (size_t i = 0; i < ad_len; i++) channel.mix_u64(ad[i]);
    CommitmentSchemeProver cs(ctx, tw, cfg);
    if (comm) { H_TRY(dist_init(ctx, comm, &cs.dist)); cs.dist.comm_ms = &st->comm_ms; cs.dist.comm_bytes = &st->comm_bytes; cs.dist.comm_calls = &st->n_alltoallv; }
    const Dist& D = cs.dist;
    for (uint32_t i = 0; i < n_comps; i++) channel.mix_u64(comps[i].log_size);
    if (host && D.on()) return set_err(ctx, NX_ERR_ARG, "nx_prove_machine_host: one GPU (a row-sharded session takes host columns through nx_prover_tree_commit_host)");
    TreeBuilder tb0 = cs.tree_builder(), tb1 = cs.tree_builder();
    GenericAir air; air.ctx = ctx;
    std::vector<DevBuf> kept[2]; kept[0].resize(n_comps); kept[1].resize(n_comps);
    std::vector<ColMap> kept_ptr[2]; kept_ptr[0].resize(n_comps); kept_ptr[1].resize(n_comps);
    auto stage_tree = [&](uint32_t tree, TreeBuilder& tb) -> int {
        std::vector<std::pair<uint32_t, uint32_t>> groups, local;
        for (uint32_t i = 0; i < n_comps; i++) groups.push_back({tree == 0 ? comps[i].n_pre : comps[i].n_main, comps[i].log_size});
        plan_local_columns(groups, D, &local);
        for (uint32_t i = 0; i < n_comps; i++) {
            const nx_component_spec& c = comps[i];
            const uint32_t lo = local[i].first, hi = local[i].second, log = c.log_size, n_tree = groups[i].first;
            DevBuf slab;
            if (host) H_TRY(slab.alloc(ctx, (size_t)n_tree << log));
            else if (hi > lo) {
                H_TRY(slab.alloc(ctx, (size_t)(hi - lo) << log));
                auto p = col_ptrs(slab.p, hi - lo, log);
                H_TRY(synth_fill_range(ctx, c, i, tree, seed, 0, lo, hi - lo, p.data(), 0, 1u << log));
            }
            const std::set<uint32_t> need = logup_needed_columns(c, tree);
            DevBuf& kb = kept[tree][i]; ColMap& kp = kept_ptr[tree][i];
            if (host) {
                std::vector<std::pair<uint32_t, uint32_t*>> keep;
                if (!need.empty()) {
                    H_TRY(kb.alloc(ctx, need.size() << log));
                    size_t q = 0;
                    for (uint32_t k : need) { uint32_t* dst = kb.p + (q++ << log); keep.push_back({k, dst}); kp[k] = dst; }
                }
                const uint32_t col0 = tree == 0 ? locs[i].pre0 : locs[i].main0;
                const uint8_t* kinds = tree == 0 ? host->pre_kinds : host->main_kinds;
                tb.extend_evals_host(std::move(slab), n_tree, log, (tree == 0 ? host->pre : host->main) + col0, kinds ? kinds + col0 : nullptr, host->coset_order, keep, col0,
                                     tree == 0 ? "nx_prove_machine_host_narrow: h_pre_cols (preprocessed trace)" : "nx_prove_machine_host_narrow: h_main_cols (main trace)");
                continue;
            }
            if (!need.empty()) {
                if (D.on() && log < (uint32_t)D.log_w + 2) return set_err(ctx, NX_ERR_ARG, "row-sharded prove: every trace column needs at least 4 rows per GPU");
                const uint64_t nb = D.on() ? D.block(log) : ((uint64_t)1 << log);
                H_TRY(kb.alloc(ctx, need.size() * (size_t)nb));
                size_t q = 0;
                std::vector<uint32_t*> cd; std::vector<const uint32_t*> csrc;
                for (uint32_t k : need) {
                    uint32_t* dst = kb.p + q * (size_t)nb;
                    if (!D.on()) { cd.push_back(dst); csrc.push_back(slab.p + ((size_t)k << log)); }
                    else { uint32_t* one[1] = {dst}; H_TRY(synth_fill_range(ctx, c, i, tree, seed, 0, k, 1, one, (uint32_t)D.begin(log), (uint32_t)nb)); }
                    kp[k] = dst; q++;
                }
                H_TRY(copy_columns(ctx, cd.data(), csrc.data(), (uint32_t)cd.size(), (size_t)nb));
            }
            tb.extend_evals_local(std::move(slab), n_tree, log, lo, hi);
        }
        return NX_OK;
    };
    std::string pre_key;
    std::shared_ptr<CommitmentTreeProver> pre_shared;
    if (ctx->opt.machine_reuse_pre && !host && !D.on()) {
        bool table = false;
        for (uint32_t i = 0; i < n_comps; i++) table = table || (comps[i].logup_mode & NX_LOGUP_TABLE);
        if (!table) {
            pre_key = "b" + std::to_string(cfg.log_blowup) + "h" + std::to_string(ctx->hash_mode);
            for (uint32_t i = 0; i < n_comps; i++) pre_key += "|" + std::to_string(comps[i].log_size) + ":" + std::to_string(comps[i].n_pre);
            auto it = ctx->machine_pre_cache.find(pre_key);
            if (it != ctx->machine_pre_cache.end()) pre_shared = std::static_pointer_cast<CommitmentTreeProver>(it->second);
        }
    }
    { HostSpan hs("pm.stage_trees(fill queued)"); if (!pre_shared) H_TRY(stage_tree(0, tb0));
    H_TRY(stage_tree(1, tb1)); }
    {
        HostSpan hs("pm.components+prepare #1");
        int rc_local = NX_OK;
        for (uint32_t i = 0; i < n_comps && rc_local == NX_OK; i++) {
            GComponent g = machine_component(comps[i], locs[i], cfg);
            g.log_cd = comps[i].log_constraint_degree_bound;
            rc_local = prepare_component_kernels(ctx, cfg, g, D.on());
            air.comps.push_back(std::move(g));
        }
        H_TRY(vote_before_exchanges(ctx, D, rc_local, "nx_prove_machine"));
    }
    lap(&st->trace_gen);
    if (pre_shared) { cs.trees.push_back(borrow_tree(pre_shared)); channel.mix_root(pre_shared->root); }
    else {
        HostSpan hs("pm.commit tree0");
        H_TRY(tb0.commit(channel));
        if (!pre_key.empty()) {
            auto sp = std::make_shared<CommitmentTreeProver>(std::move(cs.trees[0]));
            cs.trees[0] = borrow_tree(sp);
            ctx->machine_pre_cache.clear();
            ctx->machine_pre_cache[pre_key] = sp;
        }
    }
    { HostSpan hs("pm.commit tree1 (sync)"); H_TRY(tb1.commit(channel)); }
    lap(&st->commit);

    uint32_t z[4], alpha[4];
    HostSpan hs_int("pm.interaction (whole stage, host)");
    { std::vector<QM31> za = channel.draw_secure_felts(2); q_store(z, za[0]); q_store(alpha, za[1]); }
    std::vector<QM31> claimed(n_comps, q_zero());
    TreeBuilder tb2 = cs.tree_builder();
    {
        std::vector<std::pair<uint32_t, uint32_t>> groups, local;
        for (uint32_t i = 0; i < n_comps; i++) groups.push_back({comps[i].n_inter, comps[i].log_size});
        plan_local_columns(groups, D, &local);
        for (uint32_t i = 0; i < n_comps; i++) {
            const nx_component_spec& c = comps[i];
            const uint32_t log = c.log_size, L = c.n_inter / 4, lo = local[i].first, hi = local[i].second;
            DevBuf slab;
            if (L) {
                const uint32_t log_rows = D.on() ? log - (uint32_t)D.log_w : log;
                const uint64_t nb = (uint64_t)1 << log_rows;
                DevBuf rows; H_TRY(rows.alloc(ctx, (size_t)c.n_inter * nb));
                std::vector<uint32_t*> ip(c.n_inter);
                for (uint32_t k = 0; k < c.n_inter; k++) ip[k] = rows.p + (size_t)k * nb;
                { HostSpan hs("pm.logup_columns"); H_TRY(logup_columns(ctx, c, log_rows, kept_ptr[1][i], kept_ptr[0][i], z, alpha, ip.data())); }
                uint32_t cs4[4];
                if (!D.on()) {
                    { HostSpan hs("pm.logup_finalize_last (sync)"); H_TRY(nx_logup_finalize_last(ctx, log, ip.data() + 4 * (L - 1), cs4)); }
// ... 229 lines not shown
```

### nexus-zkvm_amd/csrc/prover.h

```cpp
#pragma once
#include "internal.h"
#include <memory>
#include "air.h"
#include "host/channel.h"
#include <algorithm>
#include <map>
#include <set>
#include <vector>
#include <string.h>
#include <stdlib.h>

namespace nxhip {

using namespace nx;

#define H_TRY(call) do { int rc__ = (call); if (rc__ != NX_OK) return rc__; } while (0)

struct DevBuf {
    nx_ctx* ctx = nullptr; uint32_t* p = nullptr; size_t words = 0;
    DevBuf() {}
    DevBuf(const DevBuf&) = delete;
    DevBuf& operator=(const DevBuf&) = delete;
    DevBuf(DevBuf&& o) noexcept { ctx = o.ctx; p = o.p; words = o.words; o.p = nullptr; }
    DevBuf& operator=(DevBuf&& o) noexcept { release(); ctx = o.ctx; p = o.p; words = o.words; o.p = nullptr; return *this; }
// ... 13 lines not shown
    static uint32_t cut(uint32_t n, int r, int world) { return (uint32_t)(((uint64_t)n * (uint64_t)r) / (uint64_t)world); }
    int allgather_host(nx_ctx* ctx, const void* send, size_t bytes, void* recv) const;
    int allgather_dev(nx_ctx* ctx, const uint32_t* d_send, size_t words, uint32_t* d_recv) const;
    int allgather_cols(nx_ctx* ctx, const std::vector<const uint32_t*>& blk, size_t rb, uint32_t* whole_base, uint64_t whole_stride) const;
    int alltoallv(nx_ctx* ctx, const uint32_t* d_send, const size_t* soff, const size_t* scnt, uint32_t* d_recv, const size_t* roff, const size_t* rcnt,
                  hipEvent_t ready = nullptr) const;
};
int dist_init(nx_ctx* ctx, const nx_comm* comm, Dist* out);
int vote_before_exchanges(nx_ctx* ctx, const Dist& D, int rc_local, const char* who);

struct ColumnRef { uint32_t* ptr; uint32_t log; bool block; };

struct PcsConfig { uint32_t pow_bits, log_blowup, n_queries, log_last_layer_degree_bound, fri_alpha_mode, log_constraint_degree; };
inline uint32_t comp_log_cd(uint32_t bound, const PcsConfig& cfg) { return bound ? bound : cfg.log_constraint_degree; }
inline bool comp_log_cd_ok(uint32_t bound, uint32_t cfg_lcd) { return bound <= cfg_lcd; }
struct MerkleDecommitment { std::vector<Blake2sHash> hash_witness; std::vector<uint32_t> column_witness; };

struct TreeRef {
    nx_tree* local = nullptr;
    bool borrowed = false;
    int log_w = 0;
    uint32_t n_layers = 0;
    std::vector<std::vector<Blake2sHash>> top;
    Blake2sHash root;
    TreeRef() { memset(root.w, 0, 32); }
    TreeRef(const TreeRef&) = delete;
    TreeRef& operator=(const TreeRef&) = delete;
    TreeRef(TreeRef&& o) noexcept : local(o.local), borrowed(o.borrowed), log_w(o.log_w), n_layers(o.n_layers), top(std::move(o.top)), root(o.root) { o.local = nullptr; }
    TreeRef& operator=(TreeRef&& o) noexcept { if (local && !borrowed) nx_tree_destroy(local); local = o.local; borrowed = o.borrowed; log_w = o.log_w; n_layers = o.n_layers; top = std::move(o.top); root = o.root; o.local = nullptr; return *this; }
    ~TreeRef() { if (local && !borrowed) nx_tree_destroy(local); }
};
int merkle_commit_any(nx_ctx* ctx, const Dist& dist, const uint32_t* const* d_cols, const uint32_t* logs, uint32_t n_cols, TreeRef* out);

struct GatherBatch {
    const Dist* dist = nullptr;
    std::vector<const uint32_t*> ptrs; std::vector<uint64_t> idx; std::vector<int> owner; std::vector<uint32_t> vals;
    std::vector<std::pair<size_t, uint32_t>> imm;
    size_t add(const uint32_t* p, uint64_t i, int own = -1) {
        const bool mine = own < 0 || !dist || own == dist->rank;
        ptrs.push_back(mine ? p : nullptr); idx.push_back(mine ? i : 0); owner.push_back(own);
        return ptrs.size() - 1;
    }
    size_t add_imm(uint32_t v) { ptrs.push_back(nullptr); idx.push_back(0); owner.push_back(-1); imm.push_back({ptrs.size() - 1, v}); return ptrs.size() - 1; }
    void add_column(const ColumnRef& c, uint64_t row) {
        if (c.block && dist && dist->on()) { const uint64_t blk = dist->block(c.log); add(c.ptr, row % blk, (int)(row / blk)); }
        else add(c.ptr, row);
    }
    void add_node(const TreeRef& t, uint32_t layer, uint64_t node) {
        if (t.log_w == 0) { for (int w = 0; w < 8; w++) add(nx_merkle_layer(t.local, layer), node * 8 + w); return; }
        if (layer <= (uint32_t)t.log_w) { for (int w = 0; w < 8; w++) add_imm(t.top[layer][node].w[w]); return; }
        const uint32_t ll = layer - (uint32_t)t.log_w;
        const uint64_t per = (uint64_t)1 << ll;
        for (int w = 0; w < 8; w++) add(nx_merkle_layer(t.local, ll), (node % per) * 8 + w, (int)(node / per));
    }
    int run(nx_ctx* ctx);
};
struct DecommitPlan { size_t first = 0; std::vector<uint8_t> kind; };
DecommitPlan merkle_decommit_plan(const TreeRef& tree, const std::map<uint32_t, std::vector<size_t>>& queries_per_log, std::vector<ColumnRef> cols, GatherBatch* gb);
void merkle_decommit_fill(const DecommitPlan& plan, const GatherBatch& gb, std::vector<uint32_t>* queried_values, MerkleDecommitment* d);

struct CommitmentTreeProver {
    std::vector<ColumnRef> polys;
    std::vector<int> owner;
    std::vector<ColumnRef> evals;
    std::vector<DevBuf> bufs;
    TreeRef merkle;
    Blake2sHash root;
    std::shared_ptr<CommitmentTreeProver> backing;
    CommitmentTreeProver() {}
    CommitmentTreeProver(CommitmentTreeProver&&) = default;
    CommitmentTreeProver& operator=(CommitmentTreeProver&&) = default;
    CommitmentTreeProver(const CommitmentTreeProver&) = delete;
};

class CommitmentSchemeProver;

class TreeBuilder {
  public:
    struct Group {
        DevBuf slab; uint32_t n_cols, log; bool is_evals; uint32_t lo, hi;
        std::vector<const void*> host; int coset_order = 0;
        std::vector<uint8_t> kinds; uint32_t call_col0 = 0; const char* what = nullptr;
        std::vector<std::pair<uint32_t, uint32_t*>> keep;
    };
    explicit TreeBuilder(CommitmentSchemeProver& c) : cs(c) {}
    void extend_evals(DevBuf&& slab, uint32_t n_cols, uint32_t log) { push(std::move(slab), n_cols, log, true, 0, n_cols); }
    void extend_evals_host(DevBuf&& slab, uint32_t n_cols, uint32_t log, const void* const* h_cols, const uint8_t* kinds, int coset_order,
                           const std::vector<std::pair<uint32_t, uint32_t*>>& keep, uint32_t call_col0, const char* what) {
        push(std::move(slab), n_cols, log, true, 0, n_cols);
        Group& g = groups.back();
        g.host.assign(h_cols, h_cols + n_cols); g.coset_order = coset_order; g.keep = keep;
        if (kinds) g.kinds.assign(kinds, kinds + n_cols);
        g.call_col0 = call_col0; g.what = what;
    }
    void extend_evals_local(DevBuf&& slab, uint32_t n_cols, uint32_t log, uint32_t lo, uint32_t hi) { push(std::move(slab), n_cols, log, true, lo, hi); }
    void extend_polys(DevBuf&& slab, uint32_t n_cols, uint32_t log) { push(std::move(slab), n_cols, log, false, 0, n_cols); }
    int commit(Blake2sChannel& channel) { int rc = commit_begin(); return rc != NX_OK ? rc : commit_end(channel); }
    int commit_begin();
    int commit_end(Blake2sChannel& channel);
    TreeBuilder(TreeBuilder&&) = default;
    ~TreeBuilder() { for (auto& f : feeds) (void)f->finish(); }
  private:
    void push(DevBuf&& slab, uint32_t n, uint32_t log, bool ev, uint32_t lo, uint32_t hi) { Group g; g.slab = std::move(slab); g.n_cols = n; g.log = log; g.is_evals = ev; g.lo = lo; g.hi = hi; groups.push_back(std::move(g)); }
    int commit_dist(Blake2sChannel& channel);
    CommitmentSchemeProver& cs;
    std::vector<Group> groups;
    std::vector<std::unique_ptr<nx::HostFeed>> feeds;
    bool begun = false;
    size_t tree_index = 0;
};

void plan_local_columns(const std::vector<std::pair<uint32_t, uint32_t>>& groups, const Dist& dist, std::vector<std::pair<uint32_t, uint32_t>>* out);

class CommitmentSchemeProver {
  public:
    nx_ctx* ctx; const nx_twiddles* tw; PcsConfig cfg; Dist dist;
    std::vector<CommitmentTreeProver> trees;
    CommitmentSchemeProver(nx_ctx* c, const nx_twiddles* t, PcsConfig f) : ctx(c), tw(t), cfg(f) {}
    TreeBuilder tree_builder() { return TreeBuilder(*this); }
};

CommitmentTreeProver borrow_tree(const std::shared_ptr<CommitmentTreeProver>& src);
std::vector<uint32_t*> col_ptrs(uint32_t* base, uint32_t n, uint32_t log);
int upload_owned(nx_ctx* ctx, const uint32_t* h, size_t n_words, DevBuf* out);

struct SecureColumn {
    DevBuf buf; uint32_t log = 0; uint64_t rows = 0; bool block = false; uint32_t* c[4] = {nullptr, nullptr, nullptr, nullptr};
    int alloc(nx_ctx* ctx, uint32_t l) { return alloc_rows(ctx, l, (uint64_t)1 << l, false); }
    int alloc_rows(nx_ctx* ctx, uint32_t l, uint64_t n_rows, bool is_block) {
        log = l; rows = n_rows; block = is_block;
        H_TRY(buf.alloc(ctx, (size_t)4 * n_rows)); fix(); return NX_OK;
    }
    void fix() { for (int k = 0; k < 4; k++) c[k] = buf.p + (size_t)k * rows; }
    SecureColumn() {}
    SecureColumn(SecureColumn&& o) noexcept : buf(std::move(o.buf)), log(o.log), rows(o.rows), block(o.block) { fix(); }
    SecureColumn& operator=(SecureColumn&& o) noexcept { buf = std::move(o.buf); log = o.log; rows = o.rows; block = o.block; fix(); return *this; }
};

typedef std::vector<std::vector<std::vector<QM31>>> SampledValues;
typedef std::vector<std::vector<std::vector<QPt>>> MaskPoints;

struct AirProver {
    virtual ~AirProver() {}
    virtual int compute_composition(CommitmentSchemeProver& cs, QM31 random_coeff, DevBuf* out_polys, uint32_t* out_log) = 0;
    virtual void mask_points(QPt oods, MaskPoints* points) = 0;
    virtual QM31 eval_composition_at_point(QPt point, const SampledValues& sv, QM31 random_coeff) = 0;
};

struct EvalDomainCols { std::vector<const uint32_t*> ptrs; std::vector<DevBuf> keep; };
int columns_on_eval_domain(CommitmentSchemeProver& cs, const std::vector<std::pair<uint32_t, uint32_t>>& comp_cols, uint32_t log_size, uint32_t e,
                           const std::vector<char>& masked, EvalDomainCols* out, const std::vector<char>* used = nullptr);
int composition_accumulator(CommitmentSchemeProver& cs, std::map<uint32_t, SecureColumn>& sub, uint32_t e, SecureColumn** out);
int finalize_accumulation(CommitmentSchemeProver& cs, std::map<uint32_t, SecureColumn>& sub, DevBuf* out_polys, uint32_t* out_log,
                          std::map<uint32_t, SecureColumn>* coef = nullptr);
std::vector<uint32_t> vanishing_denominators(uint32_t log_size, uint32_t e);
QM31 coset_vanishing_q(uint32_t n, QPt p);
QPt get_random_point(Blake2sChannel& ch);

struct Lap {
    nx_ctx* ctx; bool timed; double t0;
    void operator()(double* slot) { if (!timed) return; (void)nx_sync(ctx); double t = now_ms(); *slot += t - t0; t0 = t; }
};
void finish_stats(nx_ctx* ctx, nx_prove_stats* st, double t_start);


int prove_core(nx_ctx* ctx, CommitmentSchemeProver& cs, Blake2sChannel& channel, const PcsConfig& cfg, const nx_twiddles* tw, AirProver& air,
               std::vector<uint32_t>* words, nx_prove_stats* st, Lap& lap);

struct GComponent {
    uint32_t log_size = 0, n_regs = 0, n_constraints = 0;
    uint32_t log_cd = 0;
    std::vector<nx_cinstr> prog;
    std::vector<uint32_t> econsts;
    std::vector<std::pair<uint32_t, uint32_t>> cols;
    std::vector<std::vector<int>> masks;
    const nx_air_kernel* kernel = nullptr; nx_air_kernel* owned = nullptr;
    enum { ON_FULL = 0, ON_LOW = 1, ON_HALF = 2, ON_QUARTER = 3 };
    struct Part { int where = ON_FULL; bool whole = false; std::vector<uint8_t> select; std::vector<char> used; const nx_air_kernel* kernel = nullptr; };
// ... 31 lines not shown
```

### nexus-zkvm_amd/csrc/prover.hip

```cpp
#include "prover.h"
#include <chrono>
#include <memory>
#include <mutex>
#include <string>
#include <numeric>
#include <tuple>

namespace nxhip {

double now_ms() { return std::chrono::duration<double, std::milli>(std::chrono::steady_clock::now().time_since_epoch()).count(); }

#define C_TRY(call) do { if ((call) != 0) return set_err(ctx, NX_ERR_HIP, "nx_comm callback failed: " #call); } while (0)

int dist_init(nx_ctx* ctx, const nx_comm* comm, Dist* out) {
    if (!comm || comm->world < 1 || comm->rank < 0 || comm->rank >= comm->world) return set_err(ctx, NX_ERR_ARG, "nx_comm: bad rank / world");
    int lw = 0; while ((1 << lw) < comm->world) lw++;
    if ((1 << lw) != comm->world) return set_err(ctx, NX_ERR_ARG, "nx_comm: the number of GPUs of one proof must be a power of two (row blocks are subtrees)");
    if (comm->world > 1 && (!comm->allgather || !comm->alltoallv || !comm->allgather_dev)) return set_err(ctx, NX_ERR_ARG, "nx_comm: allgather, alltoallv and allgather_dev are required");
    out->comm = comm; out->rank = comm->rank; out->world = comm->world; out->log_w = lw;
    return NX_OK;
}
int vote_before_exchanges(nx_ctx* ctx, const Dist& D, int rc_local, const char* who) {
    if (!D.on()) return rc_local;
    struct Symmetric { nx_ctx* c; bool armed = true; ~Symmetric() { if (armed) c->symmetric_failure = true; } } sym{ctx};
// ... 121 lines not shown
        const bool has_prev = (uint32_t)(log + 1) < n_layers;
        static const std::vector<size_t> none;
        auto it = queries_per_log.find((uint32_t)log);
        const std::vector<size_t>& lq = it == queries_per_log.end() ? none : it->second;
        size_t pi = 0, qi = 0;
        std::vector<size_t> total;
        while (pi < last.size() || qi < lq.size()) {
            size_t node;
            if (pi < last.size() && qi < lq.size()) node = std::min(last[pi] / 2, lq[qi]);
            else if (pi < last.size()) node = last[pi] / 2;
            else node = lq[qi];
            if (has_prev) {
                for (size_t child = 2 * node; child <= 2 * node + 1; child++) {
                    if (pi < last.size() && last[pi] == child) { pi++; continue; }
                    gb->add_node(tree, (uint32_t)log + 1, child);
                    for (int w = 0; w < 8; w++) plan.kind.push_back(0);
                }
            }
            uint8_t k = 2;
            if (qi < lq.size() && lq[qi] == node) { qi++; k = 1; }
            for (auto& c : lc) { gb->add_column(c, node); plan.kind.push_back(k); }
            total.push_back(node);
        }
        last.swap(total);
    }
    return plan;
}
void merkle_decommit_fill(const DecommitPlan& plan, const GatherBatch& gb, std::vector<uint32_t>* queried_values, MerkleDecommitment* d) {
    Blake2sHash cur; int hw = 0;
    for (size_t i = 0; i < plan.kind.size(); i++) {
        const uint32_t v = gb.vals[plan.first + i];
        if (plan.kind[i] == 0) { cur.w[hw++] = v; if (hw == 8) { d->hash_witness.push_back(cur); hw = 0; } }
        else if (plan.kind[i] == 1) { if (queried_values) queried_values->push_back(v); }
        else d->column_witness.push_back(v);
    }
}

CommitmentTreeProver borrow_tree(const std::shared_ptr<CommitmentTreeProver>& src) {
    CommitmentTreeProver t;
    t.polys = src->polys; t.owner = src->owner; t.evals = src->evals;
    t.merkle.local = src->merkle.local; t.merkle.borrowed = true; t.merkle.log_w = src->merkle.log_w; t.merkle.n_layers = src->merkle.n_layers;
    t.merkle.top = src->merkle.top; t.merkle.root = src->merkle.root;
    t.root = src->root;
    t.backing = src;
    return t;
}

std::vector<uint32_t*> col_ptrs(uint32_t* base, uint32_t n, uint32_t log) {
    std::vector<uint32_t*> v(n);
    for (uint32_t i = 0; i < n; i++) v[i] = base + ((size_t)i << log);
    return v;
}

int upload_owned(nx_ctx* ctx, const uint32_t* h, size_t n_words, DevBuf* out) {
    H_TRY(out->alloc(ctx, std::max<size_t>(n_words, 4)));
    const size_t chunk = (size_t)1 << 20;
    for (size_t off = 0; off < n_words; off += chunk) {
        const size_t n = std::min(chunk, n_words - off);
        void* st = nullptr;
        H_TRY(stage(ctx, h + off, n * 4, &st));
        NX_HIP(ctx, hipMemcpyAsync(out->p + off, st, n * 4, hipMemcpyDeviceToDevice, ctx->stream));
    }
    return NX_OK;
}

void plan_local_columns(const std::vector<std::pair<uint32_t, uint32_t>>& groups, const Dist& dist, std::vector<std::pair<uint32_t, uint32_t>>* out) {
    out->assign(groups.size(), {0u, 0u});
    for (size_t g0 = 0; g0 < groups.size();) {
        size_t g1 = g0 + 1;
        while (g1 < groups.size() && groups[g1].second == groups[g0].second) g1++;
        uint32_t n_run = 0;
        for (size_t g = g0; g < g1; g++) n_run += groups[g].first;
        const uint32_t lo = Dist::cut(n_run, dist.rank, dist.world), hi = Dist::cut(n_run, dist.rank + 1, dist.world);
        uint32_t off = 0;
        for (size_t g = g0; g < g1; g++) {
            const uint32_t a = std::max(lo, off), b = std::min(hi, off + groups[g].first);
            (*out)[g] = a < b ? std::make_pair(a - off, b - off) : std::make_pair(0u, 0u);
            off += groups[g].first;
        }
        g0 = g1;
    }
}


int TreeBuilder::commit_end(Blake2sChannel& channel) {
    if (cs.dist.on()) return commit_dist(channel);
    nx_ctx* ctx = cs.ctx;
    if (!begun) return set_err(ctx, NX_ERR_ARG, "TreeBuilder::commit_end without commit_begin");
    begun = false;
    CommitmentTreeProver& t = cs.trees[tree_index];
    H_TRY(nx_merkle_root(ctx, t.merkle.local, (uint8_t*)t.root.w));
    t.merkle.root = t.root;
    for (auto& f : feeds) H_TRY(f->finish());
    feeds.clear();
    channel.mix_root(t.root);
    return NX_OK;
}

int TreeBuilder::commit_begin() {
    if (cs.dist.on()) return NX_OK;
    nx_ctx* ctx = cs.ctx;
    if (begun) return set_err(ctx, NX_ERR_ARG, "TreeBuilder::commit_begin twice");
    CommitmentTreeProver t;
    uint32_t max_el = 0, total_leaf_cols = 0;
    for (auto& g : groups) if (g.n_cols) max_el = std::max(max_el, g.log + cs.cfg.log_blowup);
    for (auto& g : groups) if (g.n_cols && g.log + cs.cfg.log_blowup == max_el) total_leaf_cols += g.n_cols;
    for (auto& g : groups) if (g.lo != 0 || g.hi != g.n_cols) return set_err(ctx, NX_ERR_ARG, "TreeBuilder: a column shard was handed to a single-GPU commitment scheme");
    TreePipe tp;
    struct PipeGuard { nx_ctx* c; TreePipe* p; ~PipeGuard() { if (p->tree) { (void)nx_sync(c); nx_tree_destroy(p->tree); p->tree = nullptr; } } } guard{ctx, &tp};
    if (total_leaf_cols) H_TRY(tree_pipe_begin(ctx, max_el, total_leaf_cols, &tp));
    std::vector<const uint32_t*> small_cols; std::vector<uint32_t> small_logs;
    for (size_t g0 = 0; g0 < groups.size();) {
        size_t g1 = g0 + 1;
        while (g1 < groups.size() && groups[g1].log == groups[g0].log && groups[g1].is_evals == groups[g0].is_evals) g1++;
        const uint32_t log = groups[g0].log, el = log + cs.cfg.log_blowup;
        const bool is_evals = groups[g0].is_evals;
        uint32_t n_run = 0;
        for (size_t g = g0; g < g1; g++) n_run += groups[g].n_cols;
        DevBuf lde;
        if (n_run) {
            H_TRY(lde.alloc(ctx, (size_t)n_run << el));
            std::vector<uint32_t*> in;
            for (size_t g = g0; g < g1; g++) { auto p = col_ptrs(groups[g].slab.p, groups[g].n_cols, log); in.insert(in.end(), p.begin(), p.end()); }
            auto out = col_ptrs(lde.p, n_run, el);
            const bool leaf = el == max_el;
            std::vector<const void*> hsrc(n_run, nullptr); std::vector<uint32_t*> keep_of(n_run, nullptr);
            std::vector<uint8_t> hkind(n_run, (uint8_t)NX_COL_U32); std::vector<uint32_t> hcall(n_run, 0);
            bool any_host = false; int coset_order = 0; const char* what = nullptr;
            {
                uint32_t off = 0;
                for (size_t g = g0; g < g1; g++) {
                    if (!groups[g].host.empty()) {
                        if (any_host && coset_order != groups[g].coset_order) return set_err(ctx, NX_ERR_ARG, "TreeBuilder: the host columns of one run must share one order");
                        any_host = true; coset_order = groups[g].coset_order;
                        for (uint32_t k = 0; k < groups[g].n_cols; k++) hsrc[off + k] = groups[g].host[k];
                        for (uint32_t k = 0; k < groups[g].n_cols; k++) hcall[off + k] = groups[g].call_col0 + k;
                        if (!groups[g].kinds.empty()) std::copy(groups[g].kinds.begin(), groups[g].kinds.end(), hkind.begin() + off);
                        if (groups[g].what) what = groups[g].what;
                        for (auto& kv : groups[g].keep) { if (kv.first >= groups[g].n_cols) return set_err(ctx, NX_ERR_ARG, "TreeBuilder: keep index outside the group"); keep_of[off + kv.first] = kv.second; }
                    }
                    off += groups[g].n_cols;
                }
            }
            HostFeed* feed = nullptr;
            if (any_host) { feeds.emplace_back(new HostFeed()); feed = feeds.back().get(); H_TRY(feed->begin(ctx, log, coset_order)); }
            const uint32_t step = any_host ? 16u : n_run;
            for (uint32_t c0 = 0; c0 < n_run; c0 += step) {
                const uint32_t nb = std::min(step, n_run - c0);
                if (any_host) {
                    for (uint32_t a = c0; a < c0 + nb;) {
                        if (!hsrc[a]) { a++; continue; }
                        uint32_t b2 = a; while (b2 < c0 + nb && hsrc[b2]) b2++;
                        hipEvent_t ready = nullptr;
                        H_TRY(feed->chunk(hsrc.data() + a, hkind.data() + a, hcall.data() + a, what, in.data() + a, b2 - a, &ready));
                        NX_HIP(ctx, hipStreamWaitEvent(ctx->stream, ready, 0));
                        a = b2;
                    }
                    for (uint32_t a = c0; a < c0 + nb; a++) if (keep_of[a]) H_TRY(nx_copy(ctx, keep_of[a], in[a], (size_t)1 << log));
                }
                if (is_evals) H_TRY(nx_lde_batch(ctx, cs.tw, in.data() + c0, nb, log, cs.cfg.log_blowup, out.data() + c0));
                else H_TRY(nx_evaluate_batch(ctx, cs.tw, (const uint32_t* const*)in.data() + c0, nb, log, cs.cfg.log_blowup, out.data() + c0));
                if (leaf) H_TRY(tree_pipe_absorb(ctx, &tp, (const uint32_t* const*)out.data() + c0, nb, false));
            }
            for (uint32_t i = 0; i < n_run; i++) {
                t.polys.push_back({in[i], log, false}); t.evals.push_back({out[i], el, false}); t.owner.push_back(-1);
                if (!leaf) { small_cols.push_back(out[i]); small_logs.push_back(el); }
            }
        }
        for (size_t g = g0; g < g1; g++) t.bufs.push_back(std::move(groups[g].slab));
        t.bufs.push_back(std::move(lde));
        g0 = g1;
    }
    t.merkle.n_layers = max_el + 1;
    if (total_leaf_cols) H_TRY(tree_pipe_finish(ctx, &tp, small_cols.data(), small_logs.data(), (uint32_t)small_cols.size(), &t.merkle.local));
    else H_TRY(nx_merkle_commit(ctx, nullptr, nullptr, 0, &t.merkle.local));
    tree_index = cs.trees.size();
    cs.trees.push_back(std::move(t));
    groups.clear();
    begun = true;
    return NX_OK;
}

static uint32_t dist_chunks(const nx_ctx* ctx, uint32_t n_run, int world, uint32_t el) {
    const uint32_t min_loc = n_run / (uint32_t)world;
    if (ctx->opt.dist_chunks > 0) return (uint32_t)std::max(1, std::min(ctx->opt.dist_chunks, (int)std::max<uint32_t>(1, min_loc)));
    if (((uint64_t)n_run << el) < ((uint64_t)1 << 27)) return 1;
    return std::max<uint32_t>(1, std::min<uint32_t>(4, min_loc / 4));
}

int TreeBuilder::commit_dist(Blake2sChannel& channel) {
    nx_ctx* ctx = cs.ctx;
    const Dist& D = cs.dist;
    const uint32_t blow = cs.cfg.log_blowup;
    CommitmentTreeProver t;
    std::vector<const uint32_t*> all_cols; std::vector<uint32_t> all_logs;
    for (size_t g0 = 0; g0 < groups.size();) {
        size_t g1 = g0 + 1;
        while (g1 < groups.size() && groups[g1].log == groups[g0].log && groups[g1].is_evals == groups[g0].is_evals) g1++;
        const uint32_t log = groups[g0].log, el = log + blow;
        const bool is_evals = groups[g0].is_evals;
        uint32_t n_run = 0;
        for (size_t g = g0; g < g1; g++) n_run += groups[g].n_cols;
        if (n_run && el < (uint32_t)D.log_w + 2) return set_err(ctx, NX_ERR_ARG, "row-sharded commit: every LDE column needs at least 4 rows per GPU");
        const uint64_t mb = D.block(el);
        if (n_run && !is_evals) {
            DevBuf lde; H_TRY(lde.alloc(ctx, (size_t)n_run << el));
            std::vector<uint32_t*> in;
            for (size_t g = g0; g < g1; g++) {
                if (groups[g].lo != 0 || groups[g].hi != groups[g].n_cols) return set_err(ctx, NX_ERR_ARG, "TreeBuilder::extend_polys: the polynomials must be on every GPU");
                auto p = col_ptrs(groups[g].slab.p, groups[g].n_cols, log); in.insert(in.end(), p.begin(), p.end());
            }
            auto out = col_ptrs(lde.p, n_run, el);
            H_TRY(nx_evaluate_batch(ctx, cs.tw, (const uint32_t* const*)in.data(), n_run, log, blow, out.data()));
            for (uint32_t i = 0; i < n_run; i++) {
                t.polys.push_back({in[i], log, false}); t.owner.push_back(-1);
                t.evals.push_back({out[i] + D.begin(el), el, true});
                all_cols.push_back(out[i] + D.begin(el)); all_logs.push_back(el);
            }
            for (size_t g = g0; g < g1; g++) t.bufs.push_back(std::move(groups[g].slab));
            t.bufs.push_back(std::move(lde));
        } else if (n_run) {
            const uint32_t lo = Dist::cut(n_run, D.rank, D.world), hi = Dist::cut(n_run, D.rank + 1, D.world), n_loc = hi - lo;
            std::vector<uint32_t*> in;
            {
                uint32_t off = 0;
                for (size_t g = g0; g < g1; g++) {
                    const uint32_t a = std::max(lo, off), b = std::min(hi, off + groups[g].n_cols);
                    const uint32_t glo = a < b ? a - off : 0, ghi = a < b ? b - off : 0;
                    if (groups[g].lo != glo || groups[g].hi != ghi) return set_err(ctx, NX_ERR_ARG, "TreeBuilder: the column shard does not match plan_local_columns");
                    auto p = col_ptrs(groups[g].slab.p, ghi - glo, log); in.insert(in.end(), p.begin(), p.end());
                    off += groups[g].n_cols;
                }
            }
            const uint32_t Q = dist_chunks(ctx, n_run, D.world, el);
            auto chunk_cols = [&](int r, uint32_t q) { const uint32_t nl = Dist::cut(n_run, r + 1, D.world) - Dist::cut(n_run, r, D.world); return Dist::cut(nl, (int)q + 1, (int)Q) - Dist::cut(nl, (int)q, (int)Q); };
            std::vector<size_t> chunk_base(Q + 1, 0);
            for (uint32_t q = 0; q < Q; q++) { size_t n = 0; for (int r = 0; r < D.world; r++) n += chunk_cols(r, q); chunk_base[q + 1] = chunk_base[q] + n; }
            DevBuf rows; H_TRY(rows.alloc(ctx, (size_t)n_run * mb));
            {
                struct Chunk { DevBuf send; hipEvent_t ev = nullptr; uint32_t n = 0; };
                std::vector<Chunk> ch(Q);
                struct EvGuard { std::vector<Chunk>& c; ~EvGuard() { for (auto& x : c) if (x.ev) (void)hipEventDestroy(x.ev); } } ev_guard{ch};
                auto exchange = [&](uint32_t q) -> int {
                    std::vector<size_t> soff(D.world), scnt(D.world), roff(D.world), rcnt(D.world);
                    size_t at = chunk_base[q];
                    for (int r = 0; r < D.world; r++) {
                        soff[r] = (size_t)r * ch[q].n * mb; scnt[r] = (size_t)ch[q].n * mb;
                        roff[r] = at * mb; rcnt[r] = (size_t)chunk_cols(r, q) * mb; at += chunk_cols(r, q);
                    }
                    H_TRY(D.alltoallv(ctx, ch[q].send.p, soff.data(), scnt.data(), rows.p, roff.data(), rcnt.data(), Q > 1 ? ch[q].ev : nullptr));
                    ch[q].send.release();
                    return NX_OK;
// ... 787 lines not shown
    (void)nx_sync(ctx);
    ctx->machine_pre_cache.clear();
}

struct SplitCache { std::mutex mu; std::map<std::pair<nx_ctx*, std::string>, std::vector<GComponent::Part>> map; };
static SplitCache& split_cache() { static SplitCache c; return c; }
static void release_split_cache(nx_ctx* ctx) {
    SplitCache& sc = split_cache();
    std::lock_guard<std::mutex> lk(sc.mu);
    for (auto it = sc.map.begin(); it != sc.map.end();) { if (it->first.first == ctx) it = sc.map.erase(it); else ++it; }
}
int prepare_component_kernels(nx_ctx* ctx, const PcsConfig& cfg, GComponent& g, bool sharded) {
    if (g.prepared) return NX_OK;
    const uint32_t bound = comp_log_cd(g.log_cd, cfg);
    const bool can_half = ctx->opt.air_half_domain && !sharded && cfg.log_blowup == 1 && g.log_size >= 4 && g.n_constraints > 0;
    const bool can_low = ctx->opt.air_degree_split && bound > 1 && bound != cfg.log_blowup && g.n_constraints > 0;
    const bool can_quarter = ctx->opt.air_quarter_domain && cfg.log_blowup == 1 && bound == 2 && g.log_size >= 4 && g.n_constraints > 0;
    if (!can_half && !can_low && !can_quarter) {
        GComponent::Part whole; whole.whole = true; whole.where = GComponent::ON_FULL;
        if (g.kernel) whole.kernel = g.kernel; else H_TRY(cached_air_kernel(ctx, g, nullptr, &whole.kernel));
        g.parts.clear(); g.parts.push_back(std::move(whole));
        g.prepared = true;
        return NX_OK;
    }
    std::string key((const char*)g.prog.data(), g.prog.size() * sizeof(nx_cinstr));
    key += "|" + std::to_string(g.cols.size()) + "|" + std::to_string(g.n_regs) + "|" + std::to_string(g.econsts.size() / 4) + "|" + std::to_string(bound) + (can_half ? "|h" : "|-") + (can_low ? "l" : "-") + (can_quarter ? (ctx->opt.air_quarter_domain >= 2 ? "Q" : "q") : "-");
    SplitCache& sc = split_cache();
    {
        std::lock_guard<std::mutex> lk(sc.mu);
        auto it = sc.map.find({ctx, key});
        if (it != sc.map.end()) { g.parts = it->second; g.prepared = true; return NX_OK; }
    }
    std::vector<uint32_t> deg;
    air_constraint_degrees(g.prog.data(), (uint32_t)g.prog.size(), g.n_regs, &deg);
    if (deg.size() != g.n_constraints) return set_err(ctx, NX_ERR_ARG, "recorded AIR: constraint count mismatch");
    int where_of[3];
    where_of[2] = GComponent::ON_FULL;
    where_of[1] = can_low ? GComponent::ON_LOW : GComponent::ON_FULL;
    where_of[0] = can_half ? GComponent::ON_HALF : where_of[1];
    std::vector<int> where_c(g.n_constraints);
    for (uint32_t j = 0; j < g.n_constraints; j++) where_c[j] = where_of[deg[j] <= 2 ? 0 : deg[j] == 3 ? 1 : 2];
    if (can_quarter) {
        std::vector<char> nb;
        air_constraint_neighbours(g.prog.data(), (uint32_t)g.prog.size(), g.n_regs, &nb);
        const bool with_neighbours = ctx->opt.air_quarter_domain >= 2;
        for (uint32_t j = 0; j < g.n_constraints; j++) if (where_c[j] == GComponent::ON_FULL && deg[j] >= 4 && deg[j] <= 5 && (with_neighbours || !nb[j])) where_c[j] = GComponent::ON_QUARTER;
    }
    std::vector<GComponent::Part> parts;
    for (int where : {GComponent::ON_HALF, GComponent::ON_LOW, GComponent::ON_QUARTER, GComponent::ON_FULL}) {
        GComponent::Part part; part.where = where; part.select.assign(g.n_constraints, 0);
        bool any = false;
        for (uint32_t j = 0; j < g.n_constraints; j++) if (where_c[j] == where) { part.select[j] = 1; any = true; }
        if (any) parts.push_back(std::move(part));
    }
    if (parts.size() == 1 && parts[0].where == GComponent::ON_FULL) {
        parts[0].whole = true; parts[0].select.clear();
        if (g.kernel) parts[0].kernel = g.kernel; else H_TRY(cached_air_kernel(ctx, g, nullptr, &parts[0].kernel));
    } else {
        for (auto& part : parts) {
            air_subset_columns(g.prog.data(), (uint32_t)g.prog.size(), g.n_regs, (uint32_t)g.cols.size(), part.select.data(), &part.used);
            bool all = true; for (uint8_t x : part.select) all = all && x;
            H_TRY(cached_air_kernel(ctx, g, all ? nullptr : part.select.data(), &part.kernel));
        }
    }
    g.parts = parts;
    {
        std::lock_guard<std::mutex> lk(sc.mu);
        sc.map.insert({{ctx, key}, parts});
    }
    g.prepared = true;
    return NX_OK;
}

__global__ void half_fix_kernel(u32* c0, u32* c1, u32* c2, u32* c3, u32 n, u32 t0, u32 t1, u32 t2, u32 t3, u32 z0) {
    if (threadIdx.x || blockIdx.x) return;
    c0[0] = m_sub(c0[0], m_mul(t0, z0)); c1[0] = m_sub(c1[0], m_mul(t1, z0)); c2[0] = m_sub(c2[0], m_mul(t2, z0)); c3[0] = m_sub(c3[0], m_mul(t3, z0));
    c0[n] = t0; c1[n] = t1; c2[n] = t2; c3[n] = t3;
}

struct HalfGroup { SecureColumn acc; uint32_t n_extra = 0; };
static int half_group_finish(nx_ctx* ctx, CommitmentSchemeProver& cs, uint32_t n, HalfGroup& hg, SecureColumn* out_coef) {
    const uint32_t N = 1u << n;
    nx_twiddles* sub_tw = nullptr;
    H_TRY(twiddles_first_half(ctx, cs.tw, n, &sub_tw));
    struct Guard { nx_twiddles* t; ~Guard() { nx_twiddles_destroy(t); } } guard{sub_tw};
    H_TRY(nx_interpolate_batch(ctx, sub_tw, hg.acc.c, 4, n));
    const Pt w = pt_from_index(circle_domain_index((int)n + 1, bitrev(N, (int)n + 1)));
    uint32_t pts[32], idx[4] = {0, 1, 2, 3}, iw[16], qw[4];
    for (int k = 0; k < 4; k++) { QPt qp; qp.x = q_from_m(w.x); qp.y = q_from_m(w.y); q_store(pts + 8 * k, qp.x); q_store(pts + 8 * k + 4, qp.y); }
    const uint32_t* polys[4] = {hg.acc.c[0], hg.acc.c[1], hg.acc.c[2], hg.acc.c[3]};
    H_TRY(nx_eval_at_points(ctx, polys, n, idx, pts, 4, iw));
    {
        const uint32_t* gp[4] = {hg.acc.c[0], hg.acc.c[1], hg.acc.c[2], hg.acc.c[3]};
        const uint64_t gi[4] = {N, N, N, N};
        H_TRY(nx_gather(ctx, gp, gi, 4, qw));
    }
    const std::vector<uint32_t> den = vanishing_denominators(n, n + 1);
    const u32 z0 = m_inv(den[0]), z1 = m_inv(den[1]);
    const u32 dz = m_inv(m_sub(z1, z0));
    u32 t[4];
    for (int k = 0; k < 4; k++) t[k] = m_mul(m_sub(qw[k], iw[4 * k]), dz);
    H_TRY(out_coef->alloc(ctx, n + 1));
    H_TRY(nx_memset_zero(ctx, out_coef->buf.p, out_coef->buf.words));
    for (int k = 0; k < 4; k++) H_TRY(nx_copy(ctx, out_coef->c[k], hg.acc.c[k], N));
    hipLaunchKernelGGL(half_fix_kernel, dim3(1), dim3(64), 0, ctx->stream, out_coef->c[0], out_coef->c[1], out_coef->c[2], out_coef->c[3], N, t[0], t[1], t[2], t[3], z0);
    if (hipGetLastError() != hipSuccess) return set_err(ctx, NX_ERR_HIP, "half_fix_kernel launch failed");
    return NX_OK;
}

__global__ void axpy_scale_kernel(u32* __restrict__ out, const u32* __restrict__ a, const u32* __restrict__ b, u32 s1, u32 s2, u32 n) {
    const u32 i = blockIdx.x * blockDim.x + threadIdx.x;
    if (i < n) out[i] = m_mul(m_add(a[i], m_mul(s1, b[i])), s2);
}
static int axpy_scale(nx_ctx* ctx, u32* out, const u32* a, const u32* b, u32 s1, u32 s2, u32 n) {
    hipLaunchKernelGGL(axpy_scale_kernel, dim3((n + 255) / 256), dim3(256), 0, ctx->stream, out, a, b, s1, s2, n);
    if (hipGetLastError() != hipSuccess) return set_err(ctx, NX_ERR_HIP, "axpy_scale_kernel launch failed");
    return NX_OK;
}

struct QuarterGroup { SecureColumn acc2n, accq, rown; };
static int quarter_group_finish(nx_ctx* ctx, CommitmentSchemeProver& cs, uint32_t n, QuarterGroup& qg, SecureColumn* out_coef) {
    const uint32_t N = 1u << n;
    nx_twiddles* qtw = nullptr;
    H_TRY(twiddles_first_part(ctx, cs.tw, n, 2, &qtw));
    struct Guard { nx_twiddles* t; ~Guard() { nx_twiddles_destroy(t); } } guard{qtw};
    H_TRY(nx_interpolate_batch(ctx, cs.tw, qg.acc2n.c, 4, n + 1));
    const std::vector<uint32_t> d4 = vanishing_denominators(n, n + 2), d2 = vanishing_denominators(n + 1, n + 2);
    const u32 z0 = m_inv(d4[0]), z1 = m_inv(d4[1]), inv_z2 = d2[0];
    SecureColumn fq, f0q, g;
    H_TRY(fq.alloc(ctx, n)); H_TRY(f0q.alloc(ctx, n)); H_TRY(g.alloc(ctx, n));
    for (int k = 0; k < 4; k++) H_TRY(axpy_scale(ctx, fq.c[k], qg.acc2n.c[k], qg.acc2n.c[k] + N, z0, 1, N));
    { const uint32_t* src[4] = {fq.c[0], fq.c[1], fq.c[2], fq.c[3]}; H_TRY(nx_evaluate_batch(ctx, qtw, src, 4, n, 0, f0q.c)); }
    for (int k = 0; k < 4; k++) H_TRY(axpy_scale(ctx, g.c[k], qg.accq.c[k], f0q.c[k], P - 1, inv_z2, N));
    H_TRY(nx_interpolate_batch(ctx, qtw, g.c, 4, n));
    const Pt w = pt_from_index(circle_domain_index((int)n + 2, bitrev(N, (int)n + 2)));
    uint32_t pts[12 * 8], idx[12], ev[12 * 4], fw[4];
    const uint32_t* polys[12];
    for (int k = 0; k < 4; k++) { polys[k] = qg.acc2n.c[k]; polys[4 + k] = qg.acc2n.c[k] + N; polys[8 + k] = g.c[k]; }
    for (int i = 0; i < 12; i++) { idx[i] = (uint32_t)i; QPt qp; qp.x = q_from_m(w.x); qp.y = q_from_m(w.y); q_store(pts + 8 * i, qp.x); q_store(pts + 8 * i + 4, qp.y); }
    H_TRY(nx_eval_at_points(ctx, polys, n, idx, pts, 12, ev));
    {
        const uint32_t* gp[4] = {qg.accq.c[0], qg.accq.c[1], qg.accq.c[2], qg.accq.c[3]};
        const uint64_t gi[4] = {N, N, N, N};
        H_TRY(nx_gather(ctx, gp, gi, 4, fw));
    }
    const u32 dz = m_inv(m_sub(z1, z0));
    u32 t[4];
    for (int k = 0; k < 4; k++) {
        const u32 f0w = m_add(ev[4 * k], m_mul(z1, ev[4 * (4 + k)]));
        const u32 gw = m_mul(m_sub(fw[k], f0w), inv_z2);
        t[k] = m_mul(m_sub(gw, ev[4 * (8 + k)]), dz);
    }
    H_TRY(out_coef->alloc(ctx, n + 2));
    H_TRY(nx_memset_zero(ctx, out_coef->buf.p, out_coef->buf.words));
    for (int k = 0; k < 4; k++) { H_TRY(nx_copy(ctx, out_coef->c[k], qg.acc2n.c[k], 2 * (size_t)N)); H_TRY(nx_copy(ctx, out_coef->c[k] + 2 * (size_t)N, g.c[k], N)); }
    hipLaunchKernelGGL(half_fix_kernel, dim3(1), dim3(64), 0, ctx->stream, out_coef->c[0] + 2 * (size_t)N, out_coef->c[1] + 2 * (size_t)N, out_coef->c[2] + 2 * (size_t)N,
                       out_coef->c[3] + 2 * (size_t)N, N, t[0], t[1], t[2], t[3], z0);
    if (hipGetLastError() != hipSuccess) return set_err(ctx, NX_ERR_HIP, "half_fix_kernel launch failed");
    H_TRY(nx_sync(ctx));
    return NX_OK;
}

int GenericAir::compute_composition(CommitmentSchemeProver& cs, QM31 random_coeff, DevBuf* out_polys, uint32_t* out_log) {
    size_t total = 0;
    for (auto& c : comps) total += c.n_constraints;
    std::vector<QM31> powers(total);
    { QM31 a = q_one(); for (size_t i = 0; i < total; i++) { powers[i] = a; a = q_mul(a, random_coeff); } }
    std::map<uint32_t, SecureColumn> sub;
    std::map<uint32_t, HalfGroup> halves;
    std::map<uint32_t, QuarterGroup> quarters;
    std::map<uint32_t, nx_twiddles*> qtw;
    struct QtwGuard { std::map<uint32_t, nx_twiddles*>& m; ~QtwGuard() { for (auto& kv : m) nx_twiddles_destroy(kv.second); } } qtw_guard{qtw};
    size_t remaining = total;
    for (auto& c : comps) {
        const uint32_t e = c.log_size + comp_log_cd(c.log_cd, cs.cfg);
        const size_t nc = c.n_constraints;
        std::vector<uint32_t> pw(4 * nc);
        for (size_t j = 0; j < nc; j++) q_store(&pw[4 * j], powers[remaining - 1 - j]);
        remaining -= nc;
        std::vector<char> masked(c.cols.size(), 0);
        for (size_t k = 0; k < c.cols.size(); k++) for (int o : c.masks[k]) if (o != 0) masked[k] = 1;
        { HostSpan hs("cc.prepare_component_kernels"); H_TRY(prepare_component_kernels(ctx, cs.cfg, c, cs.dist.on())); }
        {
            bool any_full = false;
            for (auto& part : c.parts) any_full = any_full || part.where == GComponent::ON_FULL || part.where == GComponent::ON_QUARTER;
            SecureColumn* declared = nullptr;
            if (!any_full && e > c.log_size + 1) H_TRY(composition_accumulator(cs, sub, e, &declared));
        }
        for (const GComponent::Part& part : c.parts) {
            const std::vector<char>* used = part.whole ? nullptr : &part.used;
            if (part.where == GComponent::ON_HALF) {
                const uint32_t n = c.log_size, N = 1u << n, el = n + 1;
                HalfGroup& hg = halves[n];
                if (!hg.acc.buf.p) {
                    hg.n_extra = 4;
                    H_TRY(hg.acc.alloc_rows(ctx, n, (uint64_t)N + hg.n_extra, false));
                    H_TRY(nx_memset_zero(ctx, hg.acc.buf.p, hg.acc.buf.words));
                }
                const std::vector<uint32_t> den = vanishing_denominators(n, el);
                EvalDomainCols cols;
                H_TRY(columns_on_eval_domain(cs, c.cols, n, el, masked, &cols, used));
                uint32_t* a4[4]; for (int k = 0; k < 4; k++) a4[k] = hg.acc.c[k];
                H_TRY(air_eval_rows(ctx, part.kernel, cols.ptrs.data(), c.econsts.data(), pw.data(), den.data(), n, el, a4, 0, N + hg.n_extra));
                continue;
            }
            if (part.where == GComponent::ON_QUARTER && cs.dist.on()) {
                const Dist& D = cs.dist;
                const uint32_t n = c.log_size, N = 1u << n;
                QuarterGroup& qg = quarters[n];
                if (!qg.acc2n.buf.p) {
                    H_TRY(qg.acc2n.alloc_rows(ctx, n + 1, D.block(n + 1), true)); H_TRY(nx_memset_zero(ctx, qg.acc2n.buf.p, qg.acc2n.buf.words));
                    H_TRY(qg.accq.alloc_rows(ctx, n, D.block(n), true)); H_TRY(nx_memset_zero(ctx, qg.accq.buf.p, qg.accq.buf.words));
                    H_TRY(qg.rown.alloc_rows(ctx, n, 4, false)); H_TRY(nx_memset_zero(ctx, qg.rown.buf.p, qg.rown.buf.words));
                    H_TRY(twiddles_first_part(ctx, cs.tw, n, 2, &qtw[n]));
                }
                {
                    const std::vector<uint32_t> den = vanishing_denominators(n, n + 1);
                    EvalDomainCols cols;
                    H_TRY(columns_on_eval_domain(cs, c.cols, n, n + 1, masked, &cols, used));
                    const uint64_t rb = D.begin(n + 1);
                    uint32_t* a4[4]; for (int k = 0; k < 4; k++) a4[k] = bias_rows(qg.acc2n.c[k], rb);
                    H_TRY(air_eval_rows(ctx, part.kernel, cols.ptrs.data(), c.econsts.data(), pw.data(), den.data(), n, n + 1, a4, (uint32_t)rb, (uint32_t)D.block(n + 1)));
                }
                std::vector<size_t> sel, selm;
                for (size_t k = 0; k < c.cols.size(); k++) if (!used || (k < used->size() && (*used)[k])) (masked[k] ? selm : sel).push_back(k);
                const size_t ns = sel.size(), nm = selm.size();
                std::vector<DevBuf> keep;
                std::vector<const uint32_t*> ptrs(c.cols.size(), nullptr);
                const uint64_t rbq = D.begin(n), mbq = D.block(n);
                std::vector<uint32_t*> blk;
                if (ns) H_TRY(sharded_evaluate_exchange(cs, c.cols, sel, qtw[n], n, n, &blk, &keep));
                for (size_t i = 0; i < ns; i++) ptrs[sel[i]] = bias_rows((const uint32_t*)blk[i], rbq);
                DevBuf wholem;
                if (nm) {
                    nx_twiddles* htw = nullptr;
                    H_TRY(twiddles_first_part(ctx, cs.tw, n + 1, 1, &htw));
                    struct Guard { nx_twiddles* t; ~Guard() { nx_twiddles_destroy(t); } } guard{htw};
                    std::vector<uint32_t*> bm;
                    H_TRY(sharded_evaluate_exchange(cs, c.cols, selm, htw, n, n + 1, &bm, &keep));
                    H_TRY(wholem.alloc(ctx, nm << (n + 1)));
                    std::vector<const uint32_t*> mb(bm.begin(), bm.end());
                    H_TRY(D.allgather_cols(ctx, mb, (size_t)D.block(n + 1), wholem.p, (uint64_t)1 << (n + 1)));
                    for (size_t i = 0; i < nm; i++) ptrs[selm[i]] = wholem.p + (i << (n + 1));
                }
                const std::vector<uint32_t> den = vanishing_denominators(n, n + 2);
                {
                    uint32_t* a4[4]; for (int k = 0; k < 4; k++) a4[k] = bias_rows(qg.accq.c[k], rbq);
                    H_TRY(air_eval_rows(ctx, part.kernel, ptrs.data(), c.econsts.data(), pw.data(), den.data(), n, n + 2, a4, (uint32_t)rbq, (uint32_t)mbq));
                }
                DevBuf wv; H_TRY(wv.alloc(ctx, std::max<size_t>(ns, 4)));
                if (ns) {
                    std::vector<uint32_t> mine(ns, 0), all((size_t)D.world * ns);
                    std::vector<const uint32_t*> src; std::vector<size_t> slot;
                    for (size_t i = 0; i < ns; i++)
                        if (cs.trees[c.cols[sel[i]].first].owner[c.cols[sel[i]].second] == D.rank) { src.push_back(cs.trees[c.cols[sel[i]].first].polys[c.cols[sel[i]].second].ptr); slot.push_back(i); }
                    if (!src.empty()) {
                        const Pt w = pt_from_index(circle_domain_index((int)n + 2, bitrev(N, (int)n + 2)));
                        const size_t nl = src.size();
                        std::vector<uint32_t> pidx(nl), pts(8 * nl), ev(4 * nl);
                        uint32_t pw8[8]; { QPt qp; qp.x = q_from_m(w.x); qp.y = q_from_m(w.y); q_store(pw8, qp.x); q_store(pw8 + 4, qp.y); }
                        for (size_t i = 0; i < nl; i++) { pidx[i] = (uint32_t)i; memcpy(&pts[8 * i], pw8, 32); }
                        H_TRY(nx_eval_at_points(ctx, src.data(), n, pidx.data(), pts.data(), (uint32_t)nl, ev.data()));
                        for (size_t i = 0; i < nl; i++) mine[slot[i]] = ev[4 * i];
                    }
                    H_TRY(D.allgather_host(ctx, mine.data(), ns * 4, all.data()));
                    std::vector<uint32_t> wh(ns);
                    for (size_t i = 0; i < ns; i++) wh[i] = all[(size_t)cs.trees[c.cols[sel[i]].first].owner[c.cols[sel[i]].second] * ns + i];
                    H_TRY(nx_upload(ctx, wv.p, wh.data(), ns));
                    for (size_t i = 0; i < ns; i++) ptrs[sel[i]] = bias_rows((const uint32_t*)(wv.p + i), N);
                }
                if (ns + nm) {
                    uint32_t* a4[4]; for (int k = 0; k < 4; k++) a4[k] = bias_rows(qg.rown.c[k], N);
                    H_TRY(air_eval_rows(ctx, part.kernel, ptrs.data(), c.econsts.data(), pw.data(), den.data(), n, n + 2, a4, N, 1));
                    H_TRY(nx_sync(ctx));
                }
                continue;
            }
            if (part.where == GComponent::ON_QUARTER) {
                const uint32_t n = c.log_size, N = 1u << n;
                QuarterGroup& qg = quarters[n];
                if (!qg.acc2n.buf.p) {
                    H_TRY(qg.acc2n.alloc(ctx, n + 1)); H_TRY(nx_memset_zero(ctx, qg.acc2n.buf.p, qg.acc2n.buf.words));
                    H_TRY(qg.accq.alloc_rows(ctx, n, (uint64_t)N + 4, false)); H_TRY(nx_memset_zero(ctx, qg.accq.buf.p, qg.accq.buf.words));
                    H_TRY(twiddles_first_part(ctx, cs.tw, n, 2, &qtw[n]));
                }
                {
                    const std::vector<uint32_t> den = vanishing_denominators(n, n + 1);
                    EvalDomainCols cols;
                    H_TRY(columns_on_eval_domain(cs, c.cols, n, n + 1, masked, &cols, used));
                    H_TRY(air_eval_rows(ctx, part.kernel, cols.ptrs.data(), c.econsts.data(), pw.data(), den.data(), n, n + 1, qg.acc2n.c, 0, 2 * N));
                }
                std::vector<size_t> sel, selm;
                for (size_t k = 0; k < c.cols.size(); k++) if (!used || (k < used->size() && (*used)[k])) (masked[k] ? selm : sel).push_back(k);
                const size_t ns = sel.size(), nm = selm.size();
                std::vector<const uint32_t*> src(ns), srcm(nm);
                for (size_t i = 0; i < ns; i++) src[i] = cs.trees[c.cols[sel[i]].first].polys[c.cols[sel[i]].second].ptr;
                for (size_t i = 0; i < nm; i++) srcm[i] = cs.trees[c.cols[selm[i]].first].polys[c.cols[selm[i]].second].ptr;
                DevBuf ext, extm, wv; H_TRY(ext.alloc(ctx, std::max<size_t>(ns, 1) << n)); H_TRY(wv.alloc(ctx, std::max<size_t>(ns, 4)));
                auto dst = col_ptrs(ext.p, (uint32_t)ns, n);
                if (ns) H_TRY(nx_evaluate_batch(ctx, qtw[n], src.data(), (uint32_t)ns, n, 0, dst.data()));
                std::vector<uint32_t*> dstm;
                if (nm) {
                    nx_twiddles* htw = nullptr;
                    H_TRY(twiddles_first_part(ctx, cs.tw, n + 1, 1, &htw));
                    struct Guard { nx_twiddles* t; ~Guard() { nx_twiddles_destroy(t); } } guard{htw};
                    H_TRY(extm.alloc(ctx, nm << (n + 1)));
                    dstm = col_ptrs(extm.p, (uint32_t)nm, n + 1);
                    H_TRY(nx_evaluate_batch(ctx, htw, srcm.data(), (uint32_t)nm, n, 1, dstm.data()));
                    H_TRY(nx_sync(ctx));
                }
                const std::vector<uint32_t> den = vanishing_denominators(n, n + 2);
                std::vector<const uint32_t*> ptrs(c.cols.size(), nullptr);
                for (size_t i = 0; i < ns; i++) ptrs[sel[i]] = dst[i];
                for (size_t i = 0; i < nm; i++) ptrs[selm[i]] = dstm[i];
                uint32_t* a4[4]; for (int k = 0; k < 4; k++) a4[k] = qg.accq.c[k];
                H_TRY(air_eval_rows(ctx, part.kernel, ptrs.data(), c.econsts.data(), pw.data(), den.data(), n, n + 2, a4, 0, N));
                if (ns + nm) {
                    if (ns) {
                        const Pt w = pt_from_index(circle_domain_index((int)n + 2, bitrev(N, (int)n + 2)));
                        std::vector<uint32_t> pidx(ns), pts(8 * ns), ev(4 * ns), wh(ns);
                        uint32_t pw8[8]; { QPt qp; qp.x = q_from_m(w.x); qp.y = q_from_m(w.y); q_store(pw8, qp.x); q_store(pw8 + 4, qp.y); }
                        for (size_t i = 0; i < ns; i++) { pidx[i] = (uint32_t)i; memcpy(&pts[8 * i], pw8, 32); }
                        H_TRY(nx_eval_at_points(ctx, src.data(), n, pidx.data(), pts.data(), (uint32_t)ns, ev.data()));
                        for (size_t i = 0; i < ns; i++) wh[i] = ev[4 * i];
                        H_TRY(nx_upload(ctx, wv.p, wh.data(), ns));
                        for (size_t i = 0; i < ns; i++) ptrs[sel[i]] = bias_rows((const uint32_t*)(wv.p + i), N);
                    }
                    H_TRY(air_eval_rows(ctx, part.kernel, ptrs.data(), c.econsts.data(), pw.data(), den.data(), n, n + 2, a4, N, 1));
                    H_TRY(nx_sync(ctx));
                }
                continue;
            }
            const uint32_t pe = part.where == GComponent::ON_LOW ? c.log_size + 1 : e;
            const std::vector<uint32_t> den = vanishing_denominators(c.log_size, pe);
            EvalDomainCols cols;
            H_TRY(columns_on_eval_domain(cs, c.cols, c.log_size, pe, masked, &cols, used));
            SecureColumn* acc = nullptr;
            H_TRY(composition_accumulator(cs, sub, pe, &acc));
            const uint64_t rb = cs.dist.on() ? cs.dist.begin(pe) : 0;
            uint32_t* a4[4]; for (int k = 0; k < 4; k++) a4[k] = bias_rows(acc->c[k], rb);
            H_TRY(air_eval_rows(ctx, part.kernel, cols.ptrs.data(), c.econsts.data(), pw.data(), den.data(), c.log_size, pe, a4, (uint32_t)rb, (uint32_t)acc->rows));
        }
    }
    std::map<uint32_t, SecureColumn> coef;
    { HostSpan hs("cc.half_group_finish"); for (auto& kv : halves) H_TRY(half_group_finish(ctx, cs, kv.first, kv.second, &coef[kv.first + 1])); }
    for (auto& kv : quarters) {
        SecureColumn q4;
        if (cs.dist.on()) {
            QuarterGroup& qg = kv.second;
            const uint32_t n = kv.first, N = 1u << n;
            SecureColumn w2, wq, full;
            H_TRY(gather_secure(ctx, cs.dist, qg.acc2n, &w2));
            H_TRY(gather_secure(ctx, cs.dist, qg.accq, &wq));
            H_TRY(full.alloc_rows(ctx, n, (uint64_t)N + 4, false));
            H_TRY(nx_memset_zero(ctx, full.buf.p, full.buf.words));
            for (int k = 0; k < 4; k++) { H_TRY(nx_copy(ctx, full.c[k], wq.c[k], N)); H_TRY(nx_copy(ctx, full.c[k] + N, qg.rown.c[k], 1)); }
            H_TRY(nx_sync(ctx));
            qg.acc2n = std::move(w2); qg.accq = std::move(full);
        }
        H_TRY(quarter_group_finish(ctx, cs, kv.first, kv.second, &q4));
        auto it = coef.find(kv.first + 2);
        if (it == coef.end()) { coef[kv.first + 2] = std::move(q4); continue; }
        const u32* s4[4] = {q4.c[0], q4.c[1], q4.c[2], q4.c[3]};
        H_TRY(secure_accumulate(ctx, it->second.c, s4, 1u << (kv.first + 2)));
        H_TRY(nx_sync(ctx));
    }
    HostSpan hs("cc.finalize_accumulation");
    return finalize_accumulation(cs, sub, out_polys, out_log, coef.empty() ? nullptr : &coef);
}

void GenericAir::mask_points(QPt oods, MaskPoints* points) {
    points->assign(offs.size(), {});
    std::map<std::pair<uint32_t, int>, QPt> shifted;
    for (size_t t = 0; t < offs.size(); t++) {
        points->at(t).reserve(offs[t].size());
        for (size_t c = 0; c < offs[t].size(); c++) {
            std::vector<QPt> pts;
            pts.reserve(offs[t][c].size());
            for (int o : offs[t][c]) {
                if (o == 0) { pts.push_back(oods); continue; }
                auto it = shifted.find({tree_logs[t][c], o});
                if (it == shifted.end()) {
                    const int64_t idx = ((int64_t)o * ((int64_t)1 << (31 - tree_logs[t][c]))) & 0x7fffffffLL;
                    Pt s = pt_from_index((u32)idx);
                    QPt step; step.x = q_from_m(s.x); step.y = q_from_m(s.y);
                    it = shifted.insert({{tree_logs[t][c], o}, qpt_add(oods, step)}).first;
                }
                pts.push_back(it->second);
            }
            points->at(t).push_back(std::move(pts));
        }
    }
}

QM31 GenericAir::eval_composition_at_point(QPt point, const SampledValues& sv, QM31 rc) {
    QM31 acc = q_zero();
    for (auto& c : comps) {
        const QM31 di = q_inv(coset_vanishing_q(c.log_size, point));
        std::vector<QM31> R(c.n_regs, q_zero());
        auto sampled = [&](uint32_t col, int off) {
            const uint32_t t = c.cols[col].first, i = c.cols[col].second;
            const size_t k = std::find(offs[t][i].begin(), offs[t][i].end(), off) - offs[t][i].begin();
            return sv[t][i][k];
        };
        for (auto& in : c.prog) {
            switch (in.op) {
            case NX_C_LOAD: R[in.dst] = sampled(in.a, (int)in.b); break;
            case NX_C_CONST: R[in.dst] = q_from_m(in.a); break;
            case NX_C_ADD: case NX_C_ADDE: case NX_C_ADDEB: R[in.dst] = q_add(R[in.a], R[in.b]); break;
            case NX_C_SUB: case NX_C_SUBE: R[in.dst] = q_sub(R[in.a], R[in.b]); break;
            case NX_C_MUL: case NX_C_MULE: case NX_C_MULEB: R[in.dst] = q_mul(R[in.a], R[in.b]); break;
            case NX_C_NEG: R[in.dst] = q_sub(q_zero(), R[in.a]); break;
            case NX_C_CONSTE: R[in.dst] = q_load(&c.econsts[4 * in.a]); break;
            case NX_C_LOADE: {
                QM31 v = sampled(in.a, (int)in.b);
                v = q_add(v, q_mul(sampled(in.a + 1, (int)in.b), qm(0, 1, 0, 0)));
                v = q_add(v, q_mul(sampled(in.a + 2, (int)in.b), qm(0, 0, 1, 0)));
                v = q_add(v, q_mul(sampled(in.a + 3, (int)in.b), qm(0, 0, 0, 1)));
                R[in.dst] = v; break;
            }
            case NX_C_CONSTRAINT_B: case NX_C_CONSTRAINT_E: acc = q_add(q_mul(acc, rc), q_mul(di, R[in.a])); break;
            default: break;
            }
        }
    }
    return acc;
}

}

using namespace nx;

extern "C" {

int nx_lde_batch(nx_ctx* ctx, const nx_twiddles* tw, uint32_t* const* d_cols, uint32_t n_cols, uint32_t log_size, uint32_t log_blowup,
                 uint32_t* const* d_lde) {
    NX_GUARD(ctx);
    if (n_cols == 0) return NX_OK;
    ColSet c, o;
    NX_TRY(make_colset(ctx, d_cols, n_cols, &c));
    NX_TRY(make_colset(ctx, d_lde, n_cols, &o));
    return fft_lde(ctx, tw, c, n_cols, log_size, log_blowup, o);
}

int nx_lde_commit(nx_ctx* ctx, const nx_twiddles* tw, uint32_t* const* d_cols, uint32_t n_cols, uint32_t log_size, uint32_t log_blowup,
                  uint32_t* const* d_lde, uint8_t root[32]) {
    NX_GUARD(ctx);
    NX_TRY(nx_lde_batch(ctx, tw, d_cols, n_cols, log_size, log_blowup, d_lde));
    std::vector<uint32_t> logs(n_cols, log_size + log_blowup);
    nx_tree* t = nullptr;
    NX_TRY(nx_merkle_commit(ctx, (const uint32_t* const*)d_lde, logs.data(), n_cols, &t));
    int rc = nx_merkle_root(ctx, t, root);
    nx_tree_destroy(t);
    return rc;
}

int nx_merkle_decommit(nx_ctx* ctx, const nx_tree* tree, const uint32_t* const* d_cols, const uint32_t* log_sizes, uint32_t n_cols,
                       const uint32_t* query_logs, const uint32_t* query_counts, uint32_t n_query_logs, const uint64_t* queries,
                       uint32_t** queried_values, size_t* n_queried_values, uint32_t** hash_witness, size_t* n_hashes,
                       uint32_t** column_witness, size_t* n_column_witness) {
    NX_GUARD(ctx);
    if (!ctx || !tree || (n_cols && (!d_cols || !log_sizes)) || (n_query_logs && (!query_logs || !query_counts || !queries)) || !queried_values ||
        !n_queried_values || !hash_witness || !n_hashes || !column_witness || !n_column_witness)
        return set_err(ctx, NX_ERR_ARG, "nx_merkle_decommit: NULL argument");
    const uint32_t n_layers = nx_merkle_n_layers(tree);
    std::map<uint32_t, std::vector<size_t>> qpl;
    size_t off = 0;
    for (uint32_t i = 0; i < n_query_logs; i++) {
        if (query_logs[i] >= n_layers) return set_err(ctx, NX_ERR_ARG, "nx_merkle_decommit: queried layer outside the tree");
        std::vector<size_t>& v = qpl[query_logs[i]];
        for (uint32_t k = 0; k < query_counts[i]; k++) {
            const uint64_t q = queries[off + k];
            if (q >= ((uint64_t)1 << query_logs[i]) || (!v.empty() && q <= v.back())) return set_err(ctx, NX_ERR_ARG, "nx_merkle_decommit: queries must be sorted, distinct and inside their layer");
            v.push_back((size_t)q);
        }
        off += query_counts[i];
    }
    std::vector<nxhip::ColumnRef> cols(n_cols);
    for (uint32_t i = 0; i < n_cols; i++) {
        if (log_sizes[i] >= n_layers || !d_cols[i]) return set_err(ctx, NX_ERR_ARG, "nx_merkle_decommit: column larger than the tree (or NULL)");
        cols[i] = {const_cast<uint32_t*>(d_cols[i]), log_sizes[i], false};
    }
    nxhip::TreeRef ref; ref.local = const_cast<nx_tree*>(tree); ref.n_layers = n_layers;
    struct Release { nxhip::TreeRef& r; ~Release() { r.local = nullptr; } } release{ref};
    nxhip::GatherBatch gb;
    nxhip::DecommitPlan plan = nxhip::merkle_decommit_plan(ref, qpl, cols, &gb);
    NX_TRY(gb.run(ctx));
    std::vector<uint32_t> qv; nxhip::MerkleDecommitment d;
    nxhip::merkle_decommit_fill(plan, gb, &qv, &d);
    auto dup = [](const uint32_t* src, size_t n_words) -> uint32_t* { uint32_t* p = (uint32_t*)malloc(std::max<size_t>(n_words, 1) * 4); if (p && n_words) memcpy(p, src, n_words * 4); return p; };
    uint32_t* a = dup(qv.data(), qv.size());
    uint32_t* b = dup(d.hash_witness.empty() ? nullptr : d.hash_witness[0].w, d.hash_witness.size() * 8);
    uint32_t* c = dup(d.column_witness.data(), d.column_witness.size());
    if (!a || !b || !c) { free(a); free(b); free(c); return set_err(ctx, NX_ERR_OOM, "nx_merkle_decommit: malloc failed"); }
    *queried_values = a; *n_queried_values = qv.size();
    *hash_witness = b; *n_hashes = d.hash_witness.size();
    *column_witness = c; *n_column_witness = d.column_witness.size();
    return NX_OK;
}

int nx_plan_local_columns(const uint32_t* group_n_cols, const uint32_t* group_log_sizes, uint32_t n_groups, int32_t rank, int32_t world, uint32_t* lo, uint32_t* hi) {
    if ((n_groups && (!group_n_cols || !group_log_sizes || !lo || !hi)) || world < 1 || rank < 0 || rank >= world) return set_err(nullptr, NX_ERR_ARG, "nx_plan_local_columns: bad argument");
    std::vector<std::pair<uint32_t, uint32_t>> groups(n_groups), out;
    for (uint32_t i = 0; i < n_groups; i++) groups[i] = {group_n_cols[i], group_log_sizes[i]};
    nxhip::Dist d; d.rank = rank; d.world = world;
    nxhip::plan_local_columns(groups, d, &out);
    for (uint32_t i = 0; i < n_groups; i++) { lo[i] = out[i].first; hi[i] = out[i].second; }
    return NX_OK;
}

int nx_prover_create(nx_ctx* ctx, const nx_pcs_config* cfg, uint32_t max_log_size, nx_prover** out) {
    NX_GUARD(ctx);
    if (!ctx || !cfg || !out) return set_err(ctx, NX_ERR_ARG, "nx_prover_create: NULL argument");
    if (cfg->log_blowup < 1 || cfg->log_constraint_degree < 1 || cfg->log_constraint_degree > 2 || max_log_size < 1 || max_log_size + cfg->log_constraint_degree + cfg->log_blowup > 31)
        return set_err(ctx, NX_ERR_ARG, "nx_prover_create: log_blowup >= 1, log_constraint_degree in {1,2}, 1 <= max_log_size required");
    NX_TRY(nx_ctx_set_hash_mode(ctx, (int)cfg->hash_mode));
    nx_prover* p = new nx_prover();
    p->ctx = ctx; p->ucfg = *cfg; p->max_log = max_log_size;
    p->cfg = {cfg->pow_bits, cfg->log_blowup, cfg->n_queries, cfg->log_last_layer_degree_bound, cfg->fri_alpha_mode, cfg->log_constraint_degree};
    int rc = nx_twiddles_create(ctx, max_log_size + cfg->log_constraint_degree + cfg->log_blowup - 1, &p->tw);
    if (rc != NX_OK) { delete p; return rc; }
    p->cs = new nxhip::CommitmentSchemeProver(ctx, p->tw, p->cfg);
    *out = p;
    return NX_OK;
}
// ... 284 lines not shown
```

Measured before the change: 103.9 million cycles/s.

## Cache twiddle tables across proves and keep evals via out-of-place LDE coefficients

Adds an LRU cache of full twiddle tables on the context so repeated proves at the same size reuse them, and caches derived partial twiddle tables on their parent instead of rebuilding them per quotient group. It also lets the fused LDE write the coefficients for selected columns to a separate buffer. The original evaluation slab then survives in place, which replaces the device copy previously made to keep those evaluations. The cost is extra resident device memory for cached tables and coefficient buffers, plus stream syncs when a cache entry is evicted.

```diff
diff --git a/nexus-zkvm_amd/csrc/ctx.hip b/nexus-zkvm_amd/csrc/ctx.hip
--- a/nexus-zkvm_amd/csrc/ctx.hip
+++ b/nexus-zkvm_amd/csrc/ctx.hip
@@ -320,6 +320,9 @@
     o.machine_reuse_pre = env_int("NX_MACHINE_REUSE_PREPROCESSED", 0) != 0;
     o.machine_logup_program = env_int("NX_MACHINE_LOGUP_PROGRAM", 0) != 0;
     o.trace_vec4 = env_int("NX_TRACE_VEC4", 1) != 0;
+    o.prove_table_cache = env_int("NX_PROVE_TABLE_CACHE", 1) != 0;
+    o.prove_table_cache_entries = clampi(env_int("NX_PROVE_TABLE_CACHE_ENTRIES", 4), 1, 4);
+    o.machine_clone_kept = env_int("NX_MACHINE_CLONE_KEPT", 0) != 0;
     o.host_pack_threads = clampi((int)std::thread::hardware_concurrency(), 1, 16);
     return o;
 }
@@ -349,6 +352,9 @@
     {"machine.logup_program", &nx_options::machine_logup_program, 0, 1},
     {"trace.vec4", &nx_options::trace_vec4, 0, 1},
     {"host.pack_threads", &nx_options::host_pack_threads, 1, 64},
+    {"prove.table_cache", &nx_options::prove_table_cache, 0, 1},
+    {"prove.table_cache_entries", &nx_options::prove_table_cache_entries, 1, 4},
+    {"machine.clone_kept", &nx_options::machine_clone_kept, 0, 1},
 };
 int nx_ctx_set_option(nx_ctx* ctx, const char* name, int64_t value) {
     if (!ctx || !name) return set_err(ctx, NX_ERR_ARG, "nx_ctx_set_option: NULL argument");
@@ -416,6 +422,7 @@
     (void)hipStreamSynchronize(ctx->stream);
     nxhip::machine_kernels_release(ctx);
     nx::logup_kernels_release(ctx);
+    tw_cache_release_all(ctx);
     timing_flush(ctx);
     for (auto e : ctx->event_pool) (void)hipEventDestroy(e);
     dev_cache_release(ctx);
@@ -441,7 +448,7 @@
 }
 
 int nx_sync(nx_ctx* ctx) { NX_GUARD(ctx); if (!ctx) return set_err(nullptr, NX_ERR_ARG, "nx_sync: NULL context"); NX_HIP(ctx, hipStreamSynchronize(ctx->stream)); return NX_OK; }
-int nx_ctx_trim(nx_ctx* ctx) { NX_GUARD(ctx); if (!ctx) return set_err(nullptr, NX_ERR_ARG, "nx_ctx_trim: NULL context"); NX_TRY(nx_sync(ctx)); dev_cache_release(ctx); pack_ring_release(ctx); return NX_OK; }
+int nx_ctx_trim(nx_ctx* ctx) { NX_GUARD(ctx); if (!ctx) return set_err(nullptr, NX_ERR_ARG, "nx_ctx_trim: NULL context"); NX_TRY(nx_sync(ctx)); tw_cache_release_all(ctx); dev_cache_release(ctx); pack_ring_release(ctx); return NX_OK; }
 void* nx_ctx_stream(nx_ctx* ctx) { return ctx ? (void*)ctx->stream : nullptr; }
 int nx_ctx_memory(nx_ctx* ctx, uint64_t* live_bytes, uint64_t* peak_bytes, int reset_peak) {
     if (!ctx) return set_err(nullptr, NX_ERR_ARG, "nx_ctx_memory: NULL context");
diff --git a/nexus-zkvm_amd/csrc/fft.hip b/nexus-zkvm_amd/csrc/fft.hip
--- a/nexus-zkvm_amd/csrc/fft.hip
+++ b/nexus-zkvm_amd/csrc/fft.hip
@@ -356,9 +356,14 @@
     return rc != NX_OK ? rc : rj;
 }
 
+bool fft_lde_has_coef_dst(const nx_ctx* ctx, uint32_t log_size, uint32_t log_expand) { return log_expand == 1 && log_size >= 14 && ctx->opt.fft_fused; }
 int fft_lde(nx_ctx* ctx, const nx_twiddles* tw, ColSet cols, uint32_t n_cols, uint32_t log_size, uint32_t log_expand, ColSet out) {
+    return fft_lde_coef(ctx, tw, cols, n_cols, log_size, log_expand, out, nullptr);
+}
+int fft_lde_coef(nx_ctx* ctx, const nx_twiddles* tw, ColSet cols, uint32_t n_cols, uint32_t log_size, uint32_t log_expand, ColSet out, const ColSet* coef) {
     int n = (int)(log_size + log_expand);
     NX_TRY(check_tw(ctx, tw, n));
+    if (coef && !fft_lde_has_coef_dst(ctx, log_size, log_expand)) return set_err(ctx, NX_ERR_ARG, "fft_lde: a separate coefficient set needs the fused path (blow-up 2, log_size >= 14, fft.fused)");
     tune_init();
     KTimer t(ctx, NX_T_LDE, (uint64_t)n_cols * ((8ull << log_size) + (4ull << n)));
     const u32 bc = batch_for(ctx, log_size);
@@ -369,7 +374,7 @@
         u32 nb = std::min<u32>(bc, n_cols - c0);
         streams_pick(ctx, (int)bi, ns);
         if (log_expand == 1 && log_size >= 14 && ctx->opt.fft_fused) {
-            rc = fft13_lde(ctx, tw, sub_colset(cols, c0), nb, (int)log_size, sub_colset(out, c0));
+            rc = fft13_lde(ctx, tw, sub_colset(cols, c0), sub_colset(coef ? *coef : cols, c0), nb, (int)log_size, sub_colset(out, c0));
             continue;
         }
         rc = interpolate_cols(ctx, tw, sub_colset(cols, c0), nb, (int)log_size);
@@ -479,12 +484,51 @@
     *out = t;
     return NX_OK;
 }
+int twiddles_part_acquire(nx_ctx* ctx, const nx_twiddles* tw, uint32_t n, uint32_t depth, nx_twiddles** out) {
+    *out = nullptr;
+    if (!ctx->opt.prove_table_cache) return twiddles_first_part(ctx, tw, n, depth, out);
+    const auto key = std::make_pair(n, depth);
+    auto it = tw->derived.find(key);
+    if (it != tw->derived.end()) { *out = it->second; return NX_OK; }
+    nx_twiddles* t = nullptr;
+    NX_TRY(twiddles_first_part(ctx, tw, n, depth, &t));
+    t->parent = const_cast<nx_twiddles*>(tw);
+    tw->derived[key] = t;
+    *out = t;
+    return NX_OK;
+}
+void twiddles_part_release(nx_twiddles* t) { if (t && !t->parent) nx_twiddles_destroy(t); }
+
+int tw_cache_acquire(nx_ctx* ctx, uint32_t log_half, nx_twiddles** out, bool* owned) {
+    *out = nullptr; *owned = false;
+    if (!ctx->opt.prove_table_cache) { *owned = true; return nx_twiddles_create(ctx, log_half, out); }
+    auto& c = ctx->tw_cache;
+    for (size_t i = 0; i < c.size(); i++)
+        if (c[i]->log_half == log_half) { nx_twiddles* t = c[i]; c.erase(c.begin() + i); c.insert(c.begin(), t); *out = t; return NX_OK; }
+    const size_t cap = (size_t)std::max(1, ctx->opt.prove_table_cache_entries);
+    if (c.size() >= cap) {
+        (void)hipStreamSynchronize(ctx->stream);
+        for (int i = 0; i < 3; i++) (void)hipStreamSynchronize(ctx->side[i]);
+        while (c.size() >= cap) { nx_twiddles_destroy(c.back()); c.pop_back(); }
+    }
+    nx_twiddles* t = nullptr;
+    NX_TRY(nx_twiddles_create(ctx, log_half, &t));
+    c.insert(c.begin(), t);
+    *out = t;
+    return NX_OK;
+}
+void tw_cache_release_all(nx_ctx* ctx) {
+    for (nx_twiddles* t : ctx->tw_cache) nx_twiddles_destroy(t);
+    ctx->tw_cache.clear();
+}
 }
 extern "C" {
 
 void nx_twiddles_destroy(nx_twiddles* tw) {
     NX_GUARD(tw ? tw->ctx : nullptr);
     if (!tw) return;
+    for (auto& kv : tw->derived) { kv.second->parent = nullptr; nx_twiddles_destroy(kv.second); }
+    tw->derived.clear();
     dev_free(tw->ctx, tw->d_tw); dev_free(tw->ctx, tw->d_itw); dev_free(tw->ctx, tw->d_tw2); dev_free(tw->ctx, tw->d_itw2);
     delete tw;
 }
diff --git a/nexus-zkvm_amd/csrc/fft13.hip b/nexus-zkvm_amd/csrc/fft13.hip
--- a/nexus-zkvm_amd/csrc/fft13.hip
+++ b/nexus-zkvm_amd/csrc/fft13.hip
@@ -591,18 +591,18 @@
     }
 }
 
-int fft13_lde(nx_ctx* ctx, const nx_twiddles* tw, ColSet cols, u32 n_cols, int n, ColSet out) {
+int fft13_lde(nx_ctx* ctx, const nx_twiddles* tw, ColSet cols, ColSet coef, u32 n_cols, int n, ColSet out) {
     std::vector<Plan13> plan = plan13(n, ctx->opt.fft_kmax);
     const size_t P = plan.size();
     if (P < 2) return set_err(ctx, NX_ERR_ARG, "fft13_lde: needs at least two passes");
     for (size_t i = 0; i + 1 < P; i++) {
-        Pass13 a; a.src = cols; a.dst = cols; a.tw = tw->d_itw2; a.tw_log = tw->log_half; a.n = n; a.log_in = n;
+        Pass13 a; a.src = i == 0 ? cols : coef; a.dst = coef; a.tw = tw->d_itw2; a.tw_log = tw->log_half; a.n = n; a.log_in = n;
         a.lo = plan[i].lo; a.K = plan[i].K; a.B = plan[i].B; a.scale = 0;
         a.n_cols = n_cols; a.n_groups = 0; a.tiles = 1u << (n - T13_S); a.rep_log = 0;
         NX_TRY(launch13(ctx, true, i == 0, a));
     }
     {
-        PassMid m; m.cols = cols; m.out = out; m.itw = tw->d_itw2; m.tw = tw->d_tw2; m.tw_log = tw->log_half; m.n = n;
+        PassMid m; m.cols = coef; m.out = out; m.itw = tw->d_itw2; m.tw = tw->d_tw2; m.tw_log = tw->log_half; m.n = n;
         m.lo = plan[P - 1].lo; m.K = plan[P - 1].K; m.B = plan[P - 1].B; m.scale = m_inv(1u << n); m.n_cols = n_cols; m.tiles = 1u << (n - T13_S);
         NX_TRY(launch_mid(ctx, m));
     }
diff --git a/nexus-zkvm_amd/csrc/internal.h b/nexus-zkvm_amd/csrc/internal.h
--- a/nexus-zkvm_amd/csrc/internal.h
+++ b/nexus-zkvm_amd/csrc/internal.h
@@ -33,6 +33,9 @@
     int air_degree_split;
     int trace_vec4;
     int host_pack_threads;
+    int prove_table_cache;
+    int prove_table_cache_entries;
+    int machine_clone_kept;
 };
 
 struct nx_ctx {
@@ -67,6 +70,7 @@
     bool symmetric_failure = false;
     bool comm_entered = false;
     std::map<std::string, std::shared_ptr<void>> machine_pre_cache;
+    std::vector<nx_twiddles*> tw_cache;
 };
 enum { NX_T_LDE = 0, NX_T_MERKLE = 1, NX_T_QUOT = 2, NX_T_OTHER = 3 };
 
@@ -77,6 +81,8 @@
     uint32_t* d_itw;
     uint32_t* d_tw2;
     uint32_t* d_itw2;
+    nx_twiddles* parent = nullptr;
+    mutable std::map<std::pair<uint32_t, uint32_t>, nx_twiddles*> derived;
 };
 
 struct nx_tree {
@@ -211,6 +217,10 @@
                               const uint32_t* points, const uint32_t* batch_counts, const uint32_t* col_idx, const uint32_t* values, uint32_t* const* d_out4,
                               uint64_t row_begin, uint64_t n_rows);
 int twiddles_first_part(nx_ctx* ctx, const nx_twiddles* tw, uint32_t n, uint32_t depth, nx_twiddles** out);
+int twiddles_part_acquire(nx_ctx* ctx, const nx_twiddles* tw, uint32_t n, uint32_t depth, nx_twiddles** out);
+void twiddles_part_release(nx_twiddles* t);
+int tw_cache_acquire(nx_ctx* ctx, uint32_t log_half, nx_twiddles** out, bool* owned);
+void tw_cache_release_all(nx_ctx* ctx);
 inline int twiddles_first_half(nx_ctx* ctx, const nx_twiddles* tw, uint32_t n, nx_twiddles** out) { return twiddles_first_part(ctx, tw, n, 1, out); }
 int accumulate_quotients_coeffs(nx_ctx* ctx, const nx_twiddles* tw, uint32_t log_size, uint32_t log_coef, const uint32_t* const* d_polys, uint32_t n_cols,
                                 const uint32_t random_coeff[4], uint32_t n_batches, const uint32_t* points, const uint32_t* batch_counts, const uint32_t* col_idx,
@@ -227,6 +237,10 @@
 int tree_pipe_finish(nx_ctx* ctx, TreePipe* tp, const uint32_t* const* d_small_cols, const uint32_t* small_logs, uint32_t n_small, nx_tree** out);
 int leaf_chain_launch(nx_ctx* ctx, ColSet cs, uint32_t n_cols, uint32_t col_offset, uint32_t total_cols, const uint32_t* state_in, uint32_t* state_out, uint64_t row_begin, uint64_t n_rows);
 int fft_lde(nx_ctx* ctx, const nx_twiddles* tw, ColSet cols, uint32_t n_cols, uint32_t log_size, uint32_t log_expand, ColSet out);
+int fft_lde_coef(nx_ctx* ctx, const nx_twiddles* tw, ColSet cols, uint32_t n_cols, uint32_t log_size, uint32_t log_expand, ColSet out, const ColSet* coef);
+bool fft_lde_has_coef_dst(const nx_ctx* ctx, uint32_t log_size, uint32_t log_expand);
+int lde_batch_coef(nx_ctx* ctx, const nx_twiddles* tw, uint32_t* const* d_cols, uint32_t* const* d_coef, uint32_t n_cols, uint32_t log_size, uint32_t log_blowup,
+                   uint32_t* const* d_lde);
 
 int streams_fork(nx_ctx* ctx, int n_streams);
 void streams_pick(nx_ctx* ctx, int batch_index, int n_streams);
@@ -234,7 +248,7 @@
 
 int fft13_interpolate(nx_ctx* ctx, const nx_twiddles* tw, ColSet cols, uint32_t n_cols, int n);
 int fft13_evaluate(nx_ctx* ctx, const nx_twiddles* tw, ColSet polys, uint32_t n_cols, int log_in, int n, ColSet out);
-int fft13_lde(nx_ctx* ctx, const nx_twiddles* tw, ColSet cols, uint32_t n_cols, int n, ColSet out);
+int fft13_lde(nx_ctx* ctx, const nx_twiddles* tw, ColSet cols, ColSet coef, uint32_t n_cols, int n, ColSet out);
 
 
 }
diff --git a/nexus-zkvm_amd/csrc/machine.hip b/nexus-zkvm_amd/csrc/machine.hip
--- a/nexus-zkvm_amd/csrc/machine.hip
+++ b/nexus-zkvm_amd/csrc/machine.hip
@@ -146,8 +146,9 @@
     if (timed) { (void)nx_sync(ctx); t_start = lap.t0 = now_ms(); }
 
     nx_twiddles* tw = nullptr;
-    H_TRY(nx_twiddles_create(ctx, max_log + cfg.log_constraint_degree + cfg.log_blowup - 1, &tw));
-    struct TwGuard { nx_twiddles* t; ~TwGuard() { nx_twiddles_destroy(t); } } twg{tw};
+    bool tw_owned = false;
+    H_TRY(tw_cache_acquire(ctx, max_log + cfg.log_constraint_degree + cfg.log_blowup - 1, &tw, &tw_owned));
+    struct TwGuard { nx_twiddles* t; bool owned; ~TwGuard() { if (owned) nx_twiddles_destroy(t); } } twg{tw, tw_owned};
     Blake2sChannel channel;
     for (size_t i = 0; i < ad_len; i++) channel.mix_u64(ad[i]);
     CommitmentSchemeProver cs(ctx, tw, cfg);
@@ -534,8 +535,9 @@
 
     hs_pro.stop();
     nx_twiddles* tw = nullptr;
-    { HostSpan hs("pm.twiddles_create"); H_TRY(nx_twiddles_create(ctx, max_log + cfg.log_constraint_degree + cfg.log_blowup - 1, &tw)); }
-    struct TwGuard { nx_twiddles* t; ~TwGuard() { nx_twiddles_destroy(t); } } twg{tw};
+    bool tw_owned = false;
+    { HostSpan hs("pm.twiddles_create"); H_TRY(tw_cache_acquire(ctx, max_log + cfg.log_constraint_degree + cfg.log_blowup - 1, &tw, &tw_owned)); }
+    struct TwGuard { nx_twiddles* t; bool owned; ~TwGuard() { if (owned) nx_twiddles_destroy(t); } } twg{tw, tw_owned};
     Blake2sChannel channel;
     for (size_t i = 0; i < ad_len; i++) channel.mix_u64(ad[i]);
     CommitmentSchemeProver cs(ctx, tw, cfg);
@@ -574,6 +576,12 @@
                 const uint8_t* kinds = tree == 0 ? host->pre_kinds : host->main_kinds;
                 tb.extend_evals_host(std::move(slab), n_tree, log, (tree == 0 ? host->pre : host->main) + col0, kinds ? kinds + col0 : nullptr, host->coset_order, keep, col0,
                                      tree == 0 ? "nx_prove_machine_host_narrow: h_pre_cols (preprocessed trace)" : "nx_prove_machine_host_narrow: h_main_cols (main trace)");
+                continue;
+            }
+            if (!need.empty() && !D.on() && !ctx->opt.machine_clone_kept && tb.can_keep_evals(log)) {
+                for (uint32_t k : need) kp[k] = slab.p + ((size_t)k << log);
+                tb.extend_evals_local(std::move(slab), n_tree, log, lo, hi);
+                H_TRY(tb.keep_evals(std::vector<uint32_t>(need.begin(), need.end())));
                 continue;
             }
             if (!need.empty()) {
diff --git a/nexus-zkvm_amd/csrc/prover.h b/nexus-zkvm_amd/csrc/prover.h
--- a/nexus-zkvm_amd/csrc/prover.h
+++ b/nexus-zkvm_amd/csrc/prover.h
@@ -119,6 +119,7 @@
         std::vector<const void*> host; int coset_order = 0;
         std::vector<uint8_t> kinds; uint32_t call_col0 = 0; const char* what = nullptr;
         std::vector<std::pair<uint32_t, uint32_t*>> keep;
+        std::vector<std::pair<uint32_t, uint32_t*>> coef_dst; DevBuf coef_buf;
     };
     explicit TreeBuilder(CommitmentSchemeProver& c) : cs(c) {}
     void extend_evals(DevBuf&& slab, uint32_t n_cols, uint32_t log) { push(std::move(slab), n_cols, log, true, 0, n_cols); }
@@ -131,6 +132,8 @@
         g.call_col0 = call_col0; g.what = what;
     }
     void extend_evals_local(DevBuf&& slab, uint32_t n_cols, uint32_t log, uint32_t lo, uint32_t hi) { push(std::move(slab), n_cols, log, true, lo, hi); }
+    bool can_keep_evals(uint32_t log) const;
+    int keep_evals(const std::vector<uint32_t>& cols);
     void extend_polys(DevBuf&& slab, uint32_t n_cols, uint32_t log) { push(std::move(slab), n_cols, log, false, 0, n_cols); }
     int commit(Blake2sChannel& channel) { int rc = commit_begin(); return rc != NX_OK ? rc : commit_end(channel); }
     int commit_begin();
diff --git a/nexus-zkvm_amd/csrc/prover.hip b/nexus-zkvm_amd/csrc/prover.hip
--- a/nexus-zkvm_amd/csrc/prover.hip
+++ b/nexus-zkvm_amd/csrc/prover.hip
@@ -227,6 +227,22 @@
     }
 }
 
+
+bool TreeBuilder::can_keep_evals(uint32_t log) const { return !cs.dist.on() && fft_lde_has_coef_dst(cs.ctx, log, cs.cfg.log_blowup); }
+int TreeBuilder::keep_evals(const std::vector<uint32_t>& cols) {
+    nx_ctx* ctx = cs.ctx;
+    if (groups.empty() || !groups.back().is_evals || !groups.back().host.empty() || !can_keep_evals(groups.back().log))
+        return set_err(ctx, NX_ERR_ARG, "TreeBuilder::keep_evals: needs a device-resident group of evaluations on the fused LDE path");
+    Group& g = groups.back();
+    if (cols.empty()) return NX_OK;
+    H_TRY(g.coef_buf.alloc(ctx, cols.size() << g.log));
+    size_t q = 0;
+    for (uint32_t k : cols) {
+        if (k >= g.n_cols) return set_err(ctx, NX_ERR_ARG, "TreeBuilder::keep_evals: column outside the group");
+        g.coef_dst.push_back({k, g.coef_buf.p + (q++ << g.log)});
+    }
+    return NX_OK;
+}
 
 int TreeBuilder::commit_end(Blake2sChannel& channel) {
     if (cs.dist.on()) return commit_dist(channel);
@@ -269,6 +285,16 @@
             for (size_t g = g0; g < g1; g++) { auto p = col_ptrs(groups[g].slab.p, groups[g].n_cols, log); in.insert(in.end(), p.begin(), p.end()); }
             auto out = col_ptrs(lde.p, n_run, el);
             const bool leaf = el == max_el;
+            std::vector<uint32_t*> coef(in);
+            {
+                uint32_t off = 0;
+                for (size_t g = g0; g < g1; g++) {
+                    if (!groups[g].coef_dst.empty() && !(is_evals && groups[g].host.empty() && fft_lde_has_coef_dst(ctx, log, cs.cfg.log_blowup)))
+                        return set_err(ctx, NX_ERR_ARG, "TreeBuilder: separate coefficient buffers need device-resident evaluations on the fused LDE path");
+                    for (auto& kv : groups[g].coef_dst) { if (kv.first >= groups[g].n_cols) return set_err(ctx, NX_ERR_ARG, "TreeBuilder: coefficient index outside the group"); coef[off + kv.first] = kv.second; }
+                    off += groups[g].n_cols;
+                }
+            }
             std::vector<const void*> hsrc(n_run, nullptr); std::vector<uint32_t*> keep_of(n_run, nullptr);
             std::vector<uint8_t> hkind(n_run, (uint8_t)NX_COL_U32); std::vector<uint32_t> hcall(n_run, 0);
             bool any_host = false; int coset_order = 0; const char* what = nullptr;
@@ -303,16 +329,16 @@
                     }
                     for (uint32_t a = c0; a < c0 + nb; a++) if (keep_of[a]) H_TRY(nx_copy(ctx, keep_of[a], in[a], (size_t)1 << log));
                 }
-                if (is_evals) H_TRY(nx_lde_batch(ctx, cs.tw, in.data() + c0, nb, log, cs.cfg.log_blowup, out.data() + c0));
+                if (is_evals) H_TRY(lde_batch_coef(ctx, cs.tw, in.data() + c0, coef.data() + c0, nb, log, cs.cfg.log_blowup, out.data() + c0));
                 else H_TRY(nx_evaluate_batch(ctx, cs.tw, (const uint32_t* const*)in.data() + c0, nb, log, cs.cfg.log_blowup, out.data() + c0));
                 if (leaf) H_TRY(tree_pipe_absorb(ctx, &tp, (const uint32_t* const*)out.data() + c0, nb, false));
             }
             for (uint32_t i = 0; i < n_run; i++) {
-                t.polys.push_back({in[i], log, false}); t.evals.push_back({out[i], el, false}); t.owner.push_back(-1);
+                t.polys.push_back({coef[i], log, false}); t.evals.push_back({out[i], el, false}); t.owner.push_back(-1);
                 if (!leaf) { small_cols.push_back(out[i]); small_logs.push_back(el); }
             }
         }
-        for (size_t g = g0; g < g1; g++) t.bufs.push_back(std::move(groups[g].slab));
+        for (size_t g = g0; g < g1; g++) { t.bufs.push_back(std::move(groups[g].slab)); if (groups[g].coef_buf.p) t.bufs.push_back(std::move(groups[g].coef_buf)); }
         t.bufs.push_back(std::move(lde));
         g0 = g1;
     }
@@ -1266,8 +1292,8 @@
 static int half_group_finish(nx_ctx* ctx, CommitmentSchemeProver& cs, uint32_t n, HalfGroup& hg, SecureColumn* out_coef) {
     const uint32_t N = 1u << n;
     nx_twiddles* sub_tw = nullptr;
-    H_TRY(twiddles_first_half(ctx, cs.tw, n, &sub_tw));
-    struct Guard { nx_twiddles* t; ~Guard() { nx_twiddles_destroy(t); } } guard{sub_tw};
+    H_TRY(twiddles_part_acquire(ctx, cs.tw, n, 1, &sub_tw));
+    struct Guard { nx_twiddles* t; ~Guard() { twiddles_part_release(t); } } guard{sub_tw};
     H_TRY(nx_interpolate_batch(ctx, sub_tw, hg.acc.c, 4, n));
     const Pt w = pt_from_index(circle_domain_index((int)n + 1, bitrev(N, (int)n + 1)));
     uint32_t pts[32], idx[4] = {0, 1, 2, 3}, iw[16], qw[4];
@@ -1306,8 +1332,8 @@
 static int quarter_group_finish(nx_ctx* ctx, CommitmentSchemeProver& cs, uint32_t n, QuarterGroup& qg, SecureColumn* out_coef) {
     const uint32_t N = 1u << n;
     nx_twiddles* qtw = nullptr;
-    H_TRY(twiddles_first_part(ctx, cs.tw, n, 2, &qtw));
-    struct Guard { nx_twiddles* t; ~Guard() { nx_twiddles_destroy(t); } } guard{qtw};
+    H_TRY(twiddles_part_acquire(ctx, cs.tw, n, 2, &qtw));
+    struct Guard { nx_twiddles* t; ~Guard() { twiddles_part_release(t); } } guard{qtw};
     H_TRY(nx_interpolate_batch(ctx, cs.tw, qg.acc2n.c, 4, n + 1));
     const std::vector<uint32_t> d4 = vanishing_denominators(n, n + 2), d2 = vanishing_denominators(n + 1, n + 2);
     const u32 z0 = m_inv(d4[0]), z1 = m_inv(d4[1]), inv_z2 = d2[0];
@@ -1354,7 +1380,7 @@
     std::map<uint32_t, HalfGroup> halves;
     std::map<uint32_t, QuarterGroup> quarters;
     std::map<uint32_t, nx_twiddles*> qtw;
-    struct QtwGuard { std::map<uint32_t, nx_twiddles*>& m; ~QtwGuard() { for (auto& kv : m) nx_twiddles_destroy(kv.second); } } qtw_guard{qtw};
+    struct QtwGuard { std::map<uint32_t, nx_twiddles*>& m; ~QtwGuard() { for (auto& kv : m) twiddles_part_release(kv.second); } } qtw_guard{qtw};
     size_t remaining = total;
     for (auto& c : comps) {
         const uint32_t e = c.log_size + comp_log_cd(c.log_cd, cs.cfg);
@@ -1396,7 +1422,7 @@
                     H_TRY(qg.acc2n.alloc_rows(ctx, n + 1, D.block(n + 1), true)); H_TRY(nx_memset_zero(ctx, qg.acc2n.buf.p, qg.acc2n.buf.words));
                     H_TRY(qg.accq.alloc_rows(ctx, n, D.block(n), true)); H_TRY(nx_memset_zero(ctx, qg.accq.buf.p, qg.accq.buf.words));
                     H_TRY(qg.rown.alloc_rows(ctx, n, 4, false)); H_TRY(nx_memset_zero(ctx, qg.rown.buf.p, qg.rown.buf.words));
-                    H_TRY(twiddles_first_part(ctx, cs.tw, n, 2, &qtw[n]));
+                    H_TRY(twiddles_part_acquire(ctx, cs.tw, n, 2, &qtw[n]));
                 }
                 {
                     const std::vector<uint32_t> den = vanishing_denominators(n, n + 1);
@@ -1418,8 +1444,8 @@
                 DevBuf wholem;
                 if (nm) {
                     nx_twiddles* htw = nullptr;
-                    H_TRY(twiddles_first_part(ctx, cs.tw, n + 1, 1, &htw));
-                    struct Guard { nx_twiddles* t; ~Guard() { nx_twiddles_destroy(t); } } guard{htw};
+                    H_TRY(twiddles_part_acquire(ctx, cs.tw, n + 1, 1, &htw));
+                    struct Guard { nx_twiddles* t; ~Guard() { twiddles_part_release(t); } } guard{htw};
                     std::vector<uint32_t*> bm;
                     H_TRY(sharded_evaluate_exchange(cs, c.cols, selm, htw, n, n + 1, &bm, &keep));
                     H_TRY(wholem.alloc(ctx, nm << (n + 1)));
@@ -1466,7 +1492,7 @@
                 if (!qg.acc2n.buf.p) {
                     H_TRY(qg.acc2n.alloc(ctx, n + 1)); H_TRY(nx_memset_zero(ctx, qg.acc2n.buf.p, qg.acc2n.buf.words));
                     H_TRY(qg.accq.alloc_rows(ctx, n, (uint64_t)N + 4, false)); H_TRY(nx_memset_zero(ctx, qg.accq.buf.p, qg.accq.buf.words));
-                    H_TRY(twiddles_first_part(ctx, cs.tw, n, 2, &qtw[n]));
+                    H_TRY(twiddles_part_acquire(ctx, cs.tw, n, 2, &qtw[n]));
                 }
                 {
                     const std::vector<uint32_t> den = vanishing_denominators(n, n + 1);
@@ -1486,8 +1512,8 @@
                 std::vector<uint32_t*> dstm;
                 if (nm) {
                     nx_twiddles* htw = nullptr;
-                    H_TRY(twiddles_first_part(ctx, cs.tw, n + 1, 1, &htw));
-                    struct Guard { nx_twiddles* t; ~Guard() { nx_twiddles_destroy(t); } } guard{htw};
+                    H_TRY(twiddles_part_acquire(ctx, cs.tw, n + 1, 1, &htw));
+                    struct Guard { nx_twiddles* t; ~Guard() { twiddles_part_release(t); } } guard{htw};
                     H_TRY(extm.alloc(ctx, nm << (n + 1)));
                     dstm = col_ptrs(extm.p, (uint32_t)nm, n + 1);
                     H_TRY(nx_evaluate_batch(ctx, htw, srcm.data(), (uint32_t)nm, n, 1, dstm.data()));
@@ -1615,16 +1641,27 @@
 
 using namespace nx;
 
+namespace nx {
+int lde_batch_coef(nx_ctx* ctx, const nx_twiddles* tw, uint32_t* const* d_cols, uint32_t* const* d_coef, uint32_t n_cols, uint32_t log_size, uint32_t log_blowup,
+                   uint32_t* const* d_lde) {
+    if (n_cols == 0) return NX_OK;
+    ColSet c, o, k;
+    NX_TRY(make_colset(ctx, d_cols, n_cols, &c));
+    NX_TRY(make_colset(ctx, d_lde, n_cols, &o));
+    bool same = true;
+    for (uint32_t i = 0; i < n_cols && same; i++) same = d_coef[i] == d_cols[i];
+    if (same) return fft_lde(ctx, tw, c, n_cols, log_size, log_blowup, o);
+    NX_TRY(make_colset(ctx, d_coef, n_cols, &k));
+    return fft_lde_coef(ctx, tw, c, n_cols, log_size, log_blowup, o, &k);
+}
+}
+
 extern "C" {
 
 int nx_lde_batch(nx_ctx* ctx, const nx_twiddles* tw, uint32_t* const* d_cols, uint32_t n_cols, uint32_t log_size, uint32_t log_blowup,
                  uint32_t* const* d_lde) {
     NX_GUARD(ctx);
-    if (n_cols == 0) return NX_OK;
-    ColSet c, o;
-    NX_TRY(make_colset(ctx, d_cols, n_cols, &c));
-    NX_TRY(make_colset(ctx, d_lde, n_cols, &o));
-    return fft_lde(ctx, tw, c, n_cols, log_size, log_blowup, o);
+    return lde_batch_coef(ctx, tw, d_cols, d_cols, n_cols, log_size, log_blowup, d_lde);
 }
 
 int nx_lde_commit(nx_ctx* ctx, const nx_twiddles* tw, uint32_t* const* d_cols, uint32_t n_cols, uint32_t log_size, uint32_t log_blowup,
```

Result: no change. 105.3 million cycles/s (median of 6 runs) (+1.4%).
